# Okrio/CRUSE

Measured on AMD Instinct MI355X. Metric: spectrogram frames/sec training CRUSE 16kHz 20ms-hop at 1/2/4/8 MI355X, higher is better.
Workload: dtype bf16

## Files before the change

cruse_amd/_lib.py:

```python
from __future__ import annotations

import ctypes
import os

_HERE = os.path.dirname(os.path.abspath(__file__))
LIB_PATH = os.path.join(_HERE, "libcruse_hip.so")

ABI_VERSION = 14
PREC_F32, PREC_BF16X3, PREC_BF16, PREC_F16 = 0, 1, 2, 3
PREC_BY_NAME = {"f32": PREC_F32, "bf16x3": PREC_BF16X3, "bf16": PREC_BF16, "f16": PREC_F16}
DT_F32, DT_F16, DT_BF16 = 0, 1, 2

_T = {"p": ctypes.c_void_p, "i": ctypes.c_int, "f": ctypes.c_float, "q": ctypes.c_longlong, "d": ctypes.c_double, "c": ctypes.c_char_p,
      "z": ctypes.c_size_t, "Q": ctypes.c_ulonglong}

SIGNATURES = {
    "cruse_abi_version": ("", "i"),
    "cruse_last_error": ("", "s"),
    "cruse_set_option": ("cii", "i"),
    "cruse_get_option": ("cpp", "i"),
    "cruse_stft_fwd": ("piiiipppifp", "i"),
    "cruse_istft_fwd": ("ppiiiiipp", "i"),
    "cruse_istft_bwd": ("piiiiippp", "i"),
    "cruse_conv_gather": ("ppppiiiiiiiiiiiiiiip", "i"),
    "cruse_conv_scatter2": ("ppppiiiiiiiiiiiiip", "i"),
    "cruse_conv_gather_bnstats": ("ppppiiiiiiiiiipip", "i"),
    "cruse_conv_scatter2_bnstats": ("ppppiiiiiiiiipip", "i"),
    "cruse_conv_mfma_stamps": ("p", "i"),
    "cruse_conv_plan": ("i" * 17 + "p", "i"),
    "cruse_conv_gather_bnbwd": ("pppiiiiiiiiiiiipppppipiiip", "i"),
    "cruse_conv_scatter2_bnbwd": ("pppiiiiiiiiiipppppipiiip", "i"),
    "cruse_conv_wgrad_ws_bytes": ("iii", "z"),
    "cruse_conv_gather_bnbwd_in": ("pipppppp" + "iii" + "pppp" + "pp" + "iiiiiiiiiiii" + "pppppi" + "piip", "i"),
    "cruse_conv_scatter2_bnbwd_in": ("pipppppp" + "iii" + "pppp" + "pp" + "iiiiiiiiii" + "pppppi" + "piip", "i"),
    "cruse_conv_gather_bnin": ("ppiqffpppppppppppiiiiiiiiiipip", "i"),
    "cruse_conv_scatter2_bnin": ("ppiqffpppppppppppiiiiiiiiipip", "i"),
    "cruse_conv_wgrad": ("pppiiiiiiiiiiiipp", "i"),
    "cruse_channel_sum": ("pqiipp", "i"),
    "cruse_col_sum": ("pqiipp", "i"),
    "cruse_bn_stats": ("pqiipip", "i"),
    "cruse_bn_finalize_act_fwd": ("ppiqffpppppppppqiiip", "i"),
    "cruse_bn_finalize_act_fwd_c": ("ppiqffpppppippppqiiip", "i"),
    "cruse_bn_finalize": ("pqiffppppp", "i"),
    "cruse_bn_eval_stats": ("ppifppp", "i"),
    "cruse_bn_act_fwd": ("pppppppqiiip", "i"),
    "cruse_bn_act_bwd_reduce": ("ppppppqiiipip", "i"),
    "cruse_bn_act_bwd_apply": ("pppppppiqiiiiipipppp", "i"),
    "cruse_ln_fwd": ("ppppppppqiifiqqp", "i"),
    "cruse_ln_fwd_c": ("ppppppippqiifiqqp", "i"),
    "cruse_ln_bwd": ("pppppqiipppp", "i"),
    "cruse_gemm": ("iiiiipipipipiiiip", "i"),
    "cruse_gemm_bf16_nt": ("iiipqqpqqpqpiip", "i"),
    "cruse_gemm_bf16_slab_bytes": ("iii", "z"),
    "cruse_gemm_bf16_nt_slabs": ("iiipqqpqqpqipzp", "i"),
    "cruse_gemm_bf16_nt_slabs_cat": ("ipiippqqpqqpqipzp", "i"),
    "cruse_gemm_bf16_nt_groups": ("iiiippqqppqqqpqqpqip", "i"),
    "cruse_gemm_bf16_nt_seg": ("iiippqppqqpqpiiqqp", "i"),
    "cruse_cast_bf16": ("ppqp", "i"),
    "cruse_transpose_bf16": ("pqiqpqip", "i"),
    "cruse_ktile_bf16": ("piiqppp", "i"),
    "cruse_ktile_f16": ("piiqpp", "i"),
    "cruse_gemm_f16_nt": ("iiipqqpqqpqpp", "i"),
    "cruse_gemm_nt_out16": ("iiippqqppqqpqpiip", "i"),
    "cruse_gemm_bf16_nt_atr": ("iiipqipqqpqip", "i"),
    "cruse_gemm_f16x2_nt": ("iiipqqppqqpqpp", "i"),
    "cruse_ktile_f16_split": ("piiqppp", "i"),
    "cruse_cast_bf16_split": ("pppqp", "i"),
    "cruse_gemm_bf16x3_nt": ("iiippqqppqqpqpip", "i"),
    "cruse_gru_ws_bytes": ("iii", "z"),
    "cruse_gru_plan": ("iiiiip", "i"),
    "cruse_gru_seq_fwd": ("pppppppiiiiipp", "i"),
    "cruse_gru_seq_bwd": ("pppppiiiiipp", "i"),
    "cruse_gru_seq_fwd_on": ("pppppppiiiiippip", "i"),
    "cruse_gru_seq_bwd_on": ("pppppppiiiiippip", "i"),
    "cruse_gru_seq_fwd_ex": ("ppppppppqiiiiiiipipip", "i"),
    "cruse_gru_seq_fwd_gi16": ("pippppppiiiiiipipip", "i"),
    "cruse_gru_seq_bwd_ex": ("pppppppiiiiiiiiipipip", "i"),
    "cruse_gru_gate_grads": ("pppppqiiip", "i"),
    "cruse_gru_gate_grads_bf16": ("pppppqppqiip", "i"),
    "cruse_mask_loss_fwd": ("ppppqiiffpppppp", "i"),
    "cruse_mask_apply": ("pppqiippp", "i"),
    "cruse_mask_apply_bwd": ("pppppqiiipp", "i"),
    "cruse_mask_sdnr_fwd": ("pppppqiiiffpppp", "i"),
    "cruse_sisnr_fwd": ("ppiifpppp", "i"),
    "cruse_sisnr_bwd": ("pppiifpp", "i"),
    "cruse_wave_l1_mse": ("ppqifppp", "i"),
    "cruse_deepfilter_fwd": ("ppppiiiiippp", "i"),
    "cruse_deepfilter_bwd": ("ppppppiiiiippppp", "i"),
    "cruse_sigmoid_bwd": ("pppqp", "i"),
    "cruse_axpby": ("pppffqp", "i"),
    "cruse_adam_step": ("ppppqfffffifp", "i"),
    "cruse_adam_step_guarded": ("ppppqfffffiffppipppdpp", "i"),
    "cruse_step_health": ("ppppdp", "i"),
    "cruse_sumsq": ("pqpip", "i"),
    "cruse_conv2d_nchw": ("ppppiiiiiiiiiiiiiiiiiiipiip", "i"),
    "cruse_conv2d_nchw_wgrad": ("pppiiiiiiiiiiiiiiiiiip", "i"),
    "cruse_conv2d_nchw_wgrad_ex": ("ppppiiiiiiiiiiiiiiiiiip", "i"),
    "cruse_nchw_channel_sum": ("piiipip", "i"),
    "cruse_downsum_w": ("pqiipip", "i"),
    "cruse_upsample_w": ("pqiipip", "i"),
    "cruse_bn_nchw_stats": ("piiipip", "i"),
    "cruse_bn_nchw_fwd": ("ppppppiiiipip", "i"),
    "cruse_bn_nchw_bwd": ("pppppppiiiiipppppip", "i"),
    "cruse_bn_nchw_bwd_ex": ("pppppppiiiiipiipppppip", "i"),
    "cruse_conv2d_nchw_bnbwd": ("ppp" + "iiiiiii" + "iiiiiiii" + "ii" + "pppppp" + "i" + "pip" + "ip", "i"),
    "cruse_bn_nchw_stats_ex": ("piiipiip", "i"),
    "cruse_bn_nchw_fwd_train": ("ppiffpppiiiippppppip", "i"),
    "cruse_conv2d_nchw_ex": ("ppppp" + "iiiiiii" + "iiiiiiii" + "iiii" + "p" + "pi" + "ip", "i"),
    "cruse_add_nchw": ("pppqip", "i"),
    "cruse_cast_f16": ("ppqip", "i"),
    "cruse_stft_framed": ("ppiiiiiiiiifppp", "i"),
    "cruse_istft_framed": ("ppppiiiiiiiifipp", "i"),
    "cruse_mask_ops": ("ippppqfffppp", "i"),
    "cruse_polar": ("ippppqffppp", "i"),
    "cruse_rmse": ("ppqfppp", "i"),
    "cruse_c_rmse": ("ppiqffppp", "i"),
    "cruse_sisnr_plain_finalize": ("pifppp", "i"),
    "cruse_wo_male_spec": ("pppiqqqfffppp", "i"),
    "cruse_onepole_fir": ("piififpp", "i"),
    "cruse_snr_mix": ("pppiifppppp", "i"),
    "cruse_fir_causal": ("ppqiiipp", "i"),
    "cruse_stream_create_masked": ("ppi", "i"),
    "cruse_cu_census": ("piip", "i"),
    "cruse_cu_hog": ("iQp", "i"),
    "cruse_zero": ("pzp", "i"),
    "cruse_accum_f64": ("ppip", "i"),
    "cruse_counters_add": ("piqp", "i"),
    "cruse_stream_layout": ("iiiiip", "i"),
    "cruse_stream_tables": ("pp", "i"),
    "cruse_stream_encode": ("piiiiiipppppp", "i"),
    "cruse_stream_gru": ("piiiipiippfpiippiip", "i"),
    "cruse_stream_decode": ("piiiiiippfpppp", "i"),
    "cruse_stream_packet_layout": ("iiiiip", "i"),
    "cruse_stream_encode_n": ("piiiiiiiiipppppp", "i"),
    "cruse_stream_gru_proj_n": ("piiiiiipiippfppp", "i"),
    "cruse_stream_gru_rec_n": ("piiiiiippiippiip", "i"),
    "cruse_stream_decode_n": ("piiiiiiiiippfpppp", "i"),
    "cruse_stream_gru_f16": ("piiiipiippfpiipppiip", "i"),
    "cruse_stream_gru_proj_n_f16": ("piiiiiipiippfpppp", "i"),
    "cruse_stream_gru_rec_n_f16": ("piiiiiippiipppiip", "i"),
    "cruse_stream_encode_io": ("piiiiiipippppp", "i"),
    "cruse_stream_decode_io": ("piiiiiippfpppippp", "i"),
    "cruse_stream_encode_n_io": ("piiiiiiiiipippppp", "i"),
    "cruse_stream_decode_n_io": ("piiiiiiiiippfpppippp", "i"),
    "cruse_stream_resample_in": ("piipippipp", "i"),
    "cruse_stream_resample_out": ("piipppipipp", "i"),
    "cruse_stream_resample_in_n": ("piiiipippipp", "i"),
    "cruse_stream_resample_out_n": ("piiiipppipipp", "i"),
    "cruse_si_sdr": ("ppiipp", "i"),
    "cruse_stoi_layout": ("iip", "i"),
    "cruse_stoi_ws_bytes": ("ii", "z"),
    "cruse_stoi_tables": ("pp", "i"),
    "cruse_stoi": ("ppiippzpp", "i"),
    "cruse_biquad_ws_bytes": ("iii", "z"),
    "cruse_biquad_cascade": ("ppiiiiippp", "i"),
    "cruse_fftconv_spec_bytes": ("iii", "z"),
    "cruse_fftconv_ws_bytes": ("ii", "z"),
    "cruse_fftconv_prepare": ("piippzp", "i"),
    "cruse_fftconv_apply": ("piipziippzppp", "i"),
    "cruse_peak_scale": ("ppiifpp", "i"),
    "cruse_resample_poly": ("piiippppiiipiipp", "i"),
    "cruse_assemble_clips": ("pppiiipp", "i"),
}


def _load():
    if not os.path.exists(LIB_PATH):
        raise ImportError(
            f"{LIB_PATH} not found: the CRUSE HIP library must be built for gfx950 "
            "(run `python -c 'import __graft_entry__ as g; g.build()'`). There is no CPU fallback.")
    lib = ctypes.CDLL(LIB_PATH)
    for name, (args, res) in SIGNATURES.items():
        fn = getattr(lib, name)
        fn.argtypes = [_T[c] for c in args]
        fn.restype = ctypes.c_char_p if res == "s" else _T[res]
    if lib.cruse_abi_version() != ABI_VERSION:
        raise ImportError(f"libcruse_hip.so ABI version {lib.cruse_abi_version()} != {ABI_VERSION}")
    return lib


lib = _load()


def check(rc: int) -> None:
    if rc != 0:
        msg = lib.cruse_last_error()
        raise RuntimeError(f"cruse_hip error {rc}: {msg.decode() if msg else ''}")
```

cruse_amd/config.py:

```python
from __future__ import annotations

import contextlib
import os
from dataclasses import dataclass, field, fields, replace
from typing import Dict, Optional


@dataclass
class EngineConfig:
    overlap: bool = True
    defer_mask: int = 15
    inline_mask: int = 8
    fuse_bn_stats: bool = True
    fuse_bn_bwd_stats: bool = True
    gi_x3: Optional[int] = None
    gi_f16: int = 2
    fuse_bn_fwd: bool = True
    fuse_bn_bwd_apply: bool = True
    bf16_dy: bool = True
    bf16_de: bool = True
    gi_store_f16: bool = False
    dx_atr: bool = True
    pick_launch_stream: bool = True
    lib_options: Dict[str, int] = field(default_factory=dict)

    _ENV = {"overlap": ("CRUSE_OVERLAP", lambda v: v == "1"), "defer_mask": ("CRUSE_DEFER", int), "inline_mask": ("CRUSE_INLINE", int),
            "fuse_bn_stats": ("CRUSE_FUSE_BN_STATS", lambda v: v != "0"),
            
            "fuse_bn_bwd_stats": ("CRUSE_FUSE_BN_BWD", lambda v: v != "0"), 
            "gi_x3": ("CRUSE_GI_X3", int), "gi_f16": ("CRUSE_GI_F16", int), 
             
            "fuse_bn_fwd": ("CRUSE_FUSE_BN_FWD", lambda v: v != "0"), "fuse_bn_bwd_apply": ("CRUSE_FUSE_BN_BWD_APPLY", lambda v: v != "0"), "bf16_dy": ("CRUSE_BF16_DY", lambda v: v != "0"), "bf16_de": ("CRUSE_BF16_DE", lambda v: v != "0"),
            "pick_launch_stream": ("CRUSE_PICK_LAUNCH_STREAM", lambda v: v != "0"), "gi_store_f16": ("CRUSE_GI_STORE_F16", lambda v: v != "0"),
            "dx_atr": ("CRUSE_DX_ATR", lambda v: v != "0")}
    _LIB_ENV = {"CRUSE_GRU_BWD_RS": "gru_bwd_rs", "CRUSE_GRU_FWD_LEAN": "gru_fwd_lean", "CRUSE_GRU_WLO": "gru_wlo", "CRUSE_GRU_DBG": "gru_dbg",
                "CRUSE_GRU_TF": "gru_tf", "CRUSE_GRU_POLL_FWD": "gru_poll_fwd", "CRUSE_GRU_POLL_BWD": "gru_poll_bwd", "CRUSE_CM_KINT": "cm_kint",
                "CRUSE_CM_SWAP": "cm_swap", "CRUSE_CM_NW": "cm_nw", "CRUSE_PW_VALU": "pw_valu", "CRUSE_WG_DBG": "wg_dbg",
                "CRUSE_WG_RD": "wg_rd", "CRUSE_WG_GRID": "wg_grid"}

    @classmethod
    def from_env(cls, env=None) -> "EngineConfig":
        env = os.environ if env is None else env
        kw = {}
        for name, (var, conv) in cls._ENV.items():
            if var in env:
                kw[name] = conv(env[var])
        lib = {opt: int(env[var]) for var, opt in cls._LIB_ENV.items() if var in env}
        return cls(lib_options=lib, **kw)

    def non_default(self) -> dict:
        d = EngineConfig()
        return {f.name: getattr(self, f.name) for f in fields(self) if getattr(self, f.name) != getattr(d, f.name)}

    def copy(self, **kw) -> "EngineConfig":
        return replace(self, lib_options=dict(self.lib_options), **kw)


_ACTIVE = EngineConfig()


def get() -> EngineConfig:
    return _ACTIVE


@contextlib.contextmanager
def use(cfg: EngineConfig):
    global _ACTIVE
    from . import ops
    prev = _ACTIVE
    saved = {k: ops.get_option(k) for k in cfg.lib_options}
    _ACTIVE = cfg
    for k, v in cfg.lib_options.items():
        ops.set_option(k, v)
    try:
        yield cfg
    finally:
        _ACTIVE = prev
        for k, v in saved.items():
            ops.set_option(k, v)
```

cruse_amd/csrc/pointwise.hip:

```cpp
#include "common.h"
#include <stdlib.h>

namespace {

constexpr int RED_THREADS = 1024;
constexpr int CPR_MAXG = 3;

template <typename Fn>
__device__ __forceinline__ void channel_pair_reduce(long long rows, int C, int F, double* sums, Fn fn) {
    __shared__ double c1[64 * CPR_MAXG * 4], c2[64 * CPR_MAXG * 4];
    __shared__ double s1[256], s2[256];
    const int CF = C * F, ng = CF >> 2;
    const int tid = threadIdx.x, lane = tid & 63;
    for (int c = tid; c < C; c += blockDim.x) { s1[c] = 0.0; s2[c] = 0.0; }
    for (int i = tid; i < CF; i += blockDim.x) { c1[i] = 0.0; c2[i] = 0.0; }
    __syncthreads();
    float a[CPR_MAXG][4], b[CPR_MAXG][4];
#pragma unroll
    for (int g = 0; g < CPR_MAXG; ++g)
#pragma unroll
        for (int e = 0; e < 4; ++e) { a[g][e] = b[g][e] = 0.f; }
    auto flush = [&]() {
#pragma unroll
        for (int g = 0; g < CPR_MAXG; ++g) {
            const int q = lane + 64 * g;
            if (q < ng) {
#pragma unroll
                for (int e = 0; e < 4; ++e) {
                    atomicAdd(&c1[q * 4 + e], (double)a[g][e]);
                    atomicAdd(&c2[q * 4 + e], (double)b[g][e]);
                    a[g][e] = b[g][e] = 0.f;
                }
            }
        }
    };
    const int nw = blockDim.x >> 6;
    const long long wave = (long long)blockIdx.x * nw + (tid >> 6), nwave = (long long)gridDim.x * nw;
    int n = 0;
    for (long long r = wave; r < rows; r += 2 * nwave) {
        const bool two = r + nwave < rows;
#pragma unroll
        for (int g = 0; g < CPR_MAXG; ++g) {
            const int q = lane + 64 * g;
            if (q < ng) {
                float v[4], v2[4], w[4], w2[4];
                fn(r * CF + q * 4, g, v, v2);
                if (two) fn((r + nwave) * CF + q * 4, g, w, w2);
                else {
#pragma unroll
                    for (int e = 0; e < 4; ++e) { w[e] = 0.f; w2[e] = 0.f; }
                }
#pragma unroll
                for (int e = 0; e < 4; ++e) { a[g][e] += v[e] + w[e]; b[g][e] += v2[e] + w2[e]; }
            }
        }
        n += 2;
        if (n >= 32) { flush(); n = 0; }
    }
    flush();
    __syncthreads();
    for (int i = tid; i < CF; i += blockDim.x) {
        const int c = i / F;
        atomicAdd(&s1[c], c1[i]);
        atomicAdd(&s2[c], c2[i]);
    }
    __syncthreads();
    for (int c = tid; c < C; c += blockDim.x) {
        atomicAdd(&sums[c], s1[c]);
        atomicAdd(&sums[C + c], s2[c]);
    }
}

__global__ __launch_bounds__(RED_THREADS) void bn_stats_kernel(const float* y, long long rows, int C, int F, double* sums) {
    channel_pair_reduce(rows, C, F, sums, [&](long long i, int, float (&v)[4], float (&v2)[4]) {
        const float4 t = *reinterpret_cast<const float4*>(y + i);
        v[0] = t.x; v[1] = t.y; v[2] = t.z; v[3] = t.w;
#pragma unroll
        for (int e = 0; e < 4; ++e) v2[e] = v[e] * v[e];
    });
}

__global__ void bn_finalize_kernel(const double* sums, long long count, int C, float eps, float momentum,
                                   float* mean, float* rstd, float* rmean, float* rvar) {
    const int c = blockIdx.x * blockDim.x + threadIdx.x;
    if (c >= C) return;
    const double m = sums[c] / (double)count;
    double var = sums[C + c] / (double)count - m * m;
    if (var < 0.0) var = 0.0;
    mean[c] = (float)m;
    rstd[c] = (float)(1.0 / sqrt(var + (double)eps));
    if (rmean) {
        const double unb = count > 1 ? var * (double)count / (double)(count - 1) : var;
        rmean[c] = (float)((1.0 - momentum) * rmean[c] + momentum * m);
        rvar[c] = (float)((1.0 - momentum) * rvar[c] + momentum * unb);
    }
}

__global__ void bn_eval_stats_kernel(const float* rmean, const float* rvar, int C, float eps, float* mean, float* rstd) {
    const int c = blockIdx.x * blockDim.x + threadIdx.x;
    if (c >= C) return;
    mean[c] = rmean[c];
    rstd[c] = 1.0f / sqrtf(rvar[c] + eps);
}

__global__ __launch_bounds__(256) void bn_act_fwd_kernel(const float* y, const float* mean, const float* rstd,
                                                         const float* gamma, const float* beta, const float* skip,
                                                         float* out, long long rows, int C, int F, int relu) {
    extern __shared__ float tab[];
    for (int c = threadIdx.x; c < C; c += 256) {
        tab[c] = mean[c]; tab[C + c] = rstd[c]; tab[2 * C + c] = gamma[c]; tab[3 * C + c] = beta[c];
    }
    __syncthreads();
    const int CF = C * F;
    const long long n4 = rows * CF / 4;
    for (long long i = (long long)blockIdx.x * 256 + threadIdx.x; i < n4; i += (long long)gridDim.x * 256) {
        const float4 v = reinterpret_cast<const float4*>(y)[i];
        float4 s = make_float4(0.f, 0.f, 0.f, 0.f);
        if (skip) s = reinterpret_cast<const float4*>(skip)[i];
        const int j = (int)((i * 4) % CF);
        float in[4] = {v.x, v.y, v.z, v.w};
        float sk[4] = {s.x, s.y, s.z, s.w};
        float o[4];
#pragma unroll
        for (int e = 0; e < 4; ++e) {
            const int c = (j + e) / F;
            float t = (in[e] - tab[c]) * tab[C + c] * tab[2 * C + c] + tab[3 * C + c];
            if (relu) t = fmaxf(t, 0.f);
            o[e] = t + sk[e];
        }
        reinterpret_cast<float4*>(out)[i] = make_float4(o[0], o[1], o[2], o[3]);
    }
}

__device__ __forceinline__ void store_copy4(void* base, long long elem, const float o0, const float o1, const float o2, const float o3,
                                            const int copy_f16) {
    if (copy_f16) {
        typedef __attribute__((ext_vector_type(4))) _Float16 f16x4_;
        const f16x4_ b = {(_Float16)o0, (_Float16)o1, (_Float16)o2, (_Float16)o3};
        *reinterpret_cast<f16x4_*>(reinterpret_cast<_Float16*>(base) + elem) = b;
    } else {
        typedef __attribute__((ext_vector_type(4))) __bf16 bf16x4_;
        const bf16x4_ b = {(__bf16)o0, (__bf16)o1, (__bf16)o2, (__bf16)o3};
        *reinterpret_cast<bf16x4_*>(reinterpret_cast<__bf16*>(base) + elem) = b;
    }
}

__global__ __launch_bounds__(256) void bn_fin_act_fwd_kernel(const float* y, const double* sums, int nrep, double inv_count, double unb,
                                                             float eps, float momentum, const float* gamma,
                                                             const float* beta, const float* skip, float* out, __bf16* out_bf,
                                                             float* mean_o, float* rstd_o, float* rmean, float* rvar,
                                                             long long rows, int C, int F, int relu, int copy_f16) {
    extern __shared__ float tab[];
    for (int c = threadIdx.x; c < C; c += 256) {
        double t1 = 0.0, t2 = 0.0;
        for (int r = 0; r < nrep; ++r) { t1 += sums[(long long)r * 2 * C + c]; t2 += sums[(long long)r * 2 * C + C + c]; }
        const double m = t1 * inv_count;
        double var = t2 * inv_count - m * m;
        if (var < 0.0) var = 0.0;
        const float mf = (float)m, rs = (float)(1.0 / sqrt(var + (double)eps));
        tab[c] = mf; tab[C + c] = rs; tab[2 * C + c] = gamma[c]; tab[3 * C + c] = beta[c];
        if (blockIdx.x == 0) {
            mean_o[c] = mf; rstd_o[c] = rs;
            if (rmean) {
                rmean[c] = (float)((1.0 - momentum) * rmean[c] + momentum * m);
                rvar[c] = (float)((1.0 - momentum) * rvar[c] + momentum * var * unb);
            }
        }
    }
    __syncthreads();
    const int CF = C * F;
    if (CF <= 64 * CPR_MAXG * 4) {
        const int lane = threadIdx.x & 63, ng = CF >> 2;
        float pm[CPR_MAXG][4], pr[CPR_MAXG][4], pg[CPR_MAXG][4], pb[CPR_MAXG][4];
#pragma unroll
        for (int g = 0; g < CPR_MAXG; ++g)
#pragma unroll
            for (int e = 0; e < 4; ++e) {
                const int col = (lane + 64 * g) * 4 + e;
                const int c = col < CF ? col / F : 0;
                pm[g][e] = tab[c]; pr[g][e] = tab[C + c]; pg[g][e] = tab[2 * C + c]; pb[g][e] = tab[3 * C + c];
            }
        const long long wave = (long long)blockIdx.x * 4 + (threadIdx.x >> 6), nwave = (long long)gridDim.x * 4;
        for (long long r = wave; r < rows; r += nwave) {
            float4 vv[CPR_MAXG], ss[CPR_MAXG];
            if (skip) {
#pragma unroll
                for (int g = 0; g < CPR_MAXG; ++g) {
                    const int q = lane + 64 * g;
                    if (q < ng) { vv[g] = *reinterpret_cast<const float4*>(y + r * CF + q * 4); ss[g] = *reinterpret_cast<const float4*>(skip + r * CF + q * 4); }
                }
            } else {
#pragma unroll
                for (int g = 0; g < CPR_MAXG; ++g) {
                    const int q = lane + 64 * g;
                    if (q < ng) { vv[g] = *reinterpret_cast<const float4*>(y + r * CF + q * 4); ss[g] = make_float4(0.f, 0.f, 0.f, 0.f); }
                }
            }
#pragma unroll
            for (int g = 0; g < CPR_MAXG; ++g) {
                const int q = lane + 64 * g;
                if (q < ng) {
                    const long long i = r * CF + q * 4;
                    const float in[4] = {vv[g].x, vv[g].y, vv[g].z, vv[g].w}, sk[4] = {ss[g].x, ss[g].y, ss[g].z, ss[g].w};
                    float o[4];
#pragma unroll
                    for (int e = 0; e < 4; ++e) {
                        float t = (in[e] - pm[g][e]) * pr[g][e] * pg[g][e] + pb[g][e];
                        if (relu) t = fmaxf(t, 0.f);
                        o[e] = t + sk[e];
                    }
                    *reinterpret_cast<float4*>(out + i) = make_float4(o[0], o[1], o[2], o[3]);
                    if (out_bf) store_copy4(out_bf, i, o[0], o[1], o[2], o[3], copy_f16);
                }
            }
        }
        return;
    }
    const long long n4 = rows * CF / 4;
    for (long long i = (long long)blockIdx.x * 256 + threadIdx.x; i < n4; i += (long long)gridDim.x * 256) {
        const float4 v = reinterpret_cast<const float4*>(y)[i];
        float4 s = make_float4(0.f, 0.f, 0.f, 0.f);
        if (skip) s = reinterpret_cast<const float4*>(skip)[i];
        const int j = (int)((i * 4) % CF);
        const float in[4] = {v.x, v.y, v.z, v.w};
        const float sk[4] = {s.x, s.y, s.z, s.w};
        float o[4];
#pragma unroll
        for (int e = 0; e < 4; ++e) {
            const int c = (j + e) / F;
            float t = (in[e] - tab[c]) * tab[C + c] * tab[2 * C + c] + tab[3 * C + c];
            if (relu) t = fmaxf(t, 0.f);
            o[e] = t + sk[e];
        }
        reinterpret_cast<float4*>(out)[i] = make_float4(o[0], o[1], o[2], o[3]);
        if (out_bf) store_copy4(out_bf, i * 4, o[0], o[1], o[2], o[3], copy_f16);
    }
}

__global__ __launch_bounds__(RED_THREADS) void bn_act_bwd_reduce_kernel(const float* dout, const float* y, const float* mean,
                                                                const float* rstd, const float* gamma,
                                                                const float* beta, long long rows, int C, int F,
                                                                int relu, double* sums) {
    __shared__ float tab[4][256];
    float pm[CPR_MAXG][4], pr[CPR_MAXG][4], pg[CPR_MAXG][4], pb[CPR_MAXG][4];
    const int lane = threadIdx.x & 63;
    for (int c = threadIdx.x; c < C; c += blockDim.x) {
        tab[0][c] = mean[c]; tab[1][c] = rstd[c]; tab[2][c] = gamma[c]; tab[3][c] = beta[c];
    }
    __syncthreads();
#pragma unroll
    for (int g = 0; g < CPR_MAXG; ++g)
#pragma unroll
        for (int e = 0; e < 4; ++e) {
            const int col = (lane + 64 * g) * 4 + e;
            const int c = col < C * F ? col / F : 0;
            pm[g][e] = tab[0][c]; pr[g][e] = tab[1][c]; pg[g][e] = tab[2][c]; pb[g][e] = tab[3][c];
        }
    channel_pair_reduce(rows, C, F, sums, [&](long long i, int g, float (&v)[4], float (&v2)[4]) {
        const float4 yy = *reinterpret_cast<const float4*>(y + i);
        const float4 dd = *reinterpret_cast<const float4*>(dout + i);
        const float yv[4] = {yy.x, yy.y, yy.z, yy.w}, dv[4] = {dd.x, dd.y, dd.z, dd.w};
#pragma unroll
        for (int e = 0; e < 4; ++e) {
            const float xh = (yv[e] - pm[g][e]) * pr[g][e];
            float gr = dv[e];
            if (relu && !(xh * pg[g][e] + pb[g][e] > 0.f)) gr = 0.f;
            v[e] = gr; v2[e] = gr * xh;
        }
    });
}

__global__ __launch_bounds__(256) void bn_act_bwd_apply_kernel(const float* dout, const float* y, const float* mean,
                                                               const float* rstd, const float* gamma,
                                                               const float* beta, const double* sums, int nrep, long long rows,
                                                               int C, int F, int relu, int training, float* dy, int dy_bf16,
                                                               int dout_bf16, float* dgamma, float* dbeta, float* dbias) {
    __shared__ float tab[6][256];
    const double cnt = (double)rows * F;
    const int tid = threadIdx.x, lane = tid & 63;
    const int CF = C * F, ng = CF >> 2;
    for (int c = tid; c < C; c += 256) {
        double sg = 0.0, sgx = 0.0;
        for (int r = 0; r < nrep; ++r) { sg += sums[(size_t)r * 2 * C + c]; sgx += sums[(size_t)r * 2 * C + C + c]; }
        tab[0][c] = mean[c]; tab[1][c] = rstd[c]; tab[2][c] = gamma[c]; tab[3][c] = beta[c];
        tab[4][c] = training ? (float)(sg / cnt) : 0.f;
        tab[5][c] = training ? (float)(sgx / cnt) : 0.f;
        if (blockIdx.x == 0) {
            if (dgamma) dgamma[c] += (float)sgx;
            if (dbeta) dbeta[c] += (float)sg;
            if (dbias && !training) dbias[c] += gamma[c] * rstd[c] * (float)sg;
        }
    }
    __syncthreads();
    float pm[CPR_MAXG][4], pr[CPR_MAXG][4], pg[CPR_MAXG][4], pb[CPR_MAXG][4], p1[CPR_MAXG][4], p2[CPR_MAXG][4];
#pragma unroll
    for (int g = 0; g < CPR_MAXG; ++g)
#pragma unroll
        for (int e = 0; e < 4; ++e) {
            const int col = (lane + 64 * g) * 4 + e;
            const int c = col < CF ? col / F : 0;
            pm[g][e] = tab[0][c]; pr[g][e] = tab[1][c]; pg[g][e] = tab[2][c]; pb[g][e] = tab[3][c];
            p1[g][e] = tab[4][c]; p2[g][e] = tab[5][c];
        }
    const long long wave = (long long)blockIdx.x * 4 + (tid >> 6), nwave = (long long)gridDim.x * 4;
    for (long long r = wave; r < rows; r += nwave) {
        float4 vv[CPR_MAXG], dv[CPR_MAXG];
        if (dout_bf16) {
#pragma unroll
            for (int g = 0; g < CPR_MAXG; ++g) {
                const int q = lane + 64 * g;
                if (q < ng) {
                    const long long i = r * CF + q * 4;
                    vv[g] = *reinterpret_cast<const float4*>(y + i);
                    const float2 w2 = *reinterpret_cast<const float2*>(reinterpret_cast<const __bf16*>(dout) + i);
                    const unsigned w0 = __float_as_uint(w2.x), w1 = __float_as_uint(w2.y);
                    dv[g] = make_float4(__uint_as_float(w0 << 16), __uint_as_float(w0 & 0xffff0000u), __uint_as_float(w1 << 16),
                                        __uint_as_float(w1 & 0xffff0000u));
                }
            }
        } else {
#pragma unroll
            for (int g = 0; g < CPR_MAXG; ++g) {
                const int q = lane + 64 * g;
                if (q < ng) {
                    const long long i = r * CF + q * 4;
                    vv[g] = *reinterpret_cast<const float4*>(y + i);
                    dv[g] = *reinterpret_cast<const float4*>(dout + i);
                }
            }
        }
#pragma unroll
        for (int g = 0; g < CPR_MAXG; ++g) {
            const int q = lane + 64 * g;
            if (q < ng) {
                const long long i = r * CF + q * 4;
                const float in[4] = {vv[g].x, vv[g].y, vv[g].z, vv[g].w}, dd[4] = {dv[g].x, dv[g].y, dv[g].z, dv[g].w};
                float o[4];
#pragma unroll
                for (int e = 0; e < 4; ++e) {
                    const float xh = (in[e] - pm[g][e]) * pr[g][e];
                    float gr = dd[e];
                    if (relu && !(xh * pg[g][e] + pb[g][e] > 0.f)) gr = 0.f;
                    o[e] = pg[g][e] * pr[g][e] * (gr - p1[g][e] - xh * p2[g][e]);
                }
                if (dy_bf16) {
                    typedef __attribute__((ext_vector_type(4))) __bf16 bf16x4_;
                    bf16x4_ h;
                    h[0] = (__bf16)o[0]; h[1] = (__bf16)o[1]; h[2] = (__bf16)o[2]; h[3] = (__bf16)o[3];
                    *reinterpret_cast<bf16x4_*>(reinterpret_cast<__bf16*>(dy) + i) = h;
                } else {
                    *reinterpret_cast<float4*>(dy + i) = make_float4(o[0], o[1], o[2], o[3]);
                }
            }
        }
    }
}

constexpr int LN_MAXE = 16;

__device__ __forceinline__ int ln_perm(int c, int H, int g) {
    if (g <= 1) return c;
    const int Hg = H / g;
    return (c % Hg) * g + c / Hg;
}

__global__ __launch_bounds__(256) void ln_fwd_kernel(const float* x, const float* gamma, const float* beta,
                                                     const float* res, float* y, float* mean, float* rstd,
                                                     long long rows, int H, int g, float eps) {
    const int lane = threadIdx.x & 63;
    const long long wave = (long long)blockIdx.x * 4 + (threadIdx.x >> 6);
    const long long nwave = (long long)gridDim.x * 4;
    for (long long r = wave; r < rows; r += nwave) {
        float v[LN_MAXE];
        float s = 0.f;
#pragma unroll
        for (int e = 0; e < LN_MAXE; ++e) {
            const int c = lane + 64 * e;
            v[e] = c < H ? x[r * H + c] : 0.f;
            s += v[e];
        }
        const float m = wave_sum(s) / (float)H;
        float q = 0.f;
#pragma unroll
        for (int e = 0; e < LN_MAXE; ++e) {
            const int c = lane + 64 * e;
            const float d = c < H ? v[e] - m : 0.f;
            q += d * d;
        }
        const float rs = 1.0f / sqrtf(wave_sum(q) / (float)H + eps);
        if (lane == 0) { if (mean) mean[r] = m; if (rstd) rstd[r] = rs; }
#pragma unroll
        for (int e = 0; e < LN_MAXE; ++e) {
            const int c = lane + 64 * e;
            if (c < H) {
                const int p = ln_perm(c, H, g);
                float o = (v[e] - m) * rs * gamma[p] + beta[p];
                if (res) o += res[r * H + p];
                y[r * H + p] = o;
            }
        }
    }
}

__global__ __launch_bounds__(256) void ln_bwd_kernel(const float* dy, const float* x, const float* mean,
                                                     const float* rstd, const float* gamma, long long rows, int H,
                                                     int g, float* dx, float* dgamma, float* dbeta) {
    __shared__ float sdg[1024], sdb[1024];
    const int lane = threadIdx.x & 63;
    for (int c = threadIdx.x; c < H; c += 256) { sdg[c] = 0.f; sdb[c] = 0.f; }
    __syncthreads();
    const long long wave = (long long)blockIdx.x * 4 + (threadIdx.x >> 6);
    const long long nwave = (long long)gridDim.x * 4;
    float adg[LN_MAXE], adb[LN_MAXE];
    int perm[LN_MAXE];
    float gm[LN_MAXE];
#pragma unroll
    for (int e = 0; e < LN_MAXE; ++e) {
        adg[e] = 0.f; adb[e] = 0.f;
        const int c = lane + 64 * e;
        perm[e] = c < H ? ln_perm(c, H, g) : 0;
        gm[e] = c < H ? gamma[perm[e]] : 0.f;
    }
    for (long long r = wave; r < rows; r += nwave) {
        const float m = mean[r], rs = rstd[r];
        float xh[LN_MAXE], gd[LN_MAXE];
        float s1 = 0.f, s2 = 0.f;
#pragma unroll
        for (int e = 0; e < LN_MAXE; ++e) {
            const int c = lane + 64 * e;
            if (c < H) {
                const float d = dy[r * H + perm[e]];
                xh[e] = (x[r * H + c] - m) * rs;
                gd[e] = d * gm[e];
                adg[e] += d * xh[e];
                adb[e] += d;
                s1 += gd[e];
                s2 += gd[e] * xh[e];
            } else { xh[e] = 0.f; gd[e] = 0.f; }
        }
        const float m1 = wave_sum(s1) / (float)H, m2 = wave_sum(s2) / (float)H;
#pragma unroll
        for (int e = 0; e < LN_MAXE; ++e) {
            const int c = lane + 64 * e;
            if (c < H) dx[r * H + c] = rs * (gd[e] - m1 - xh[e] * m2);
        }
    }
#pragma unroll
    for (int e = 0; e < LN_MAXE; ++e) {
        const int c = lane + 64 * e;
        if (c < H) { atomicAdd(&sdg[perm[e]], adg[e]); atomicAdd(&sdb[perm[e]], adb[e]); }
    }
    __syncthreads();
    for (int c = threadIdx.x; c < H; c += 256) {
        if (dgamma) atomicAdd(&dgamma[c], sdg[c]);
        if (dbeta) atomicAdd(&dbeta[c], sdb[c]);
    }
}

constexpr int LNV_MAXQ = 4;
constexpr int LNV_NR = 2;

struct RowSeg { int len; long long stride, off; };
__device__ __forceinline__ long long seg_row(const RowSeg& sg, long long r) {
    if (sg.len == 0) return r;
    const long long q = r / sg.len;
    return q * sg.stride + sg.off + (r - q * sg.len);
}

__global__ __launch_bounds__(256) void ln_fwd_vec_kernel(const float* x, const float* gamma, const float* beta,
                                                         const float* res, float* y, __bf16* y_bf, float* mean, float* rstd,
                                                         long long rows, int H, float eps, RowSeg sg, int copy_f16) {
    const int lane = threadIdx.x & 63, nq = H >> 2;
    const long long wave = (long long)blockIdx.x * 4 + (threadIdx.x >> 6);
    const long long nwave = (long long)gridDim.x * 4;
    float4 gm[LNV_MAXQ], bt[LNV_MAXQ];
#pragma unroll
    for (int e = 0; e < LNV_MAXQ; ++e) {
        const int q = lane + 64 * e;
        gm[e] = q < nq ? reinterpret_cast<const float4*>(gamma)[q] : make_float4(0.f, 0.f, 0.f, 0.f);
        bt[e] = q < nq ? reinterpret_cast<const float4*>(beta)[q] : make_float4(0.f, 0.f, 0.f, 0.f);
    }
    for (long long r0 = wave * LNV_NR; r0 < rows; r0 += nwave * LNV_NR) {
        float4 v[LNV_NR][LNV_MAXQ], rv[LNV_NR][LNV_MAXQ];
        float s[LNV_NR], m[LNV_NR], qq[LNV_NR];
#pragma unroll
        for (int k = 0; k < LNV_NR; ++k) {
            const long long rl = r0 + k, r = seg_row(sg, rl < rows ? rl : rows - 1);
            s[k] = 0.f;
#pragma unroll
            for (int e = 0; e < LNV_MAXQ; ++e) {
                const int q = lane + 64 * e;
                const bool ok = q < nq && rl < rows;
                v[k][e] = ok ? reinterpret_cast<const float4*>(x + r * H)[q] : make_float4(0.f, 0.f, 0.f, 0.f);
                rv[k][e] = (ok && res) ? reinterpret_cast<const float4*>(res + r * H)[q] : make_float4(0.f, 0.f, 0.f, 0.f);
                s[k] += (v[k][e].x + v[k][e].y) + (v[k][e].z + v[k][e].w);
            }
// ... 161 lines not shown

__global__ void sigmoid_bwd_kernel(const float* dmask, const float* mask, float* dlogit, long long n) {
    for (long long i = (long long)blockIdx.x * blockDim.x + threadIdx.x; i < n; i += (long long)gridDim.x * blockDim.x) {
        const float m = mask[i];
        dlogit[i] = dmask[i] * m * (1.f - m);
    }
}

__global__ void axpby_kernel(float* out, const float* x, const float* y, float a, float b, long long n) {
    for (long long i = (long long)blockIdx.x * blockDim.x + threadIdx.x; i < n; i += (long long)gridDim.x * blockDim.x)
        out[i] = a * x[i] + (y ? b * y[i] : 0.f);
}

__global__ void accum_f64_kernel(double* acc, const double* x, int n) {
    const int i = blockIdx.x * blockDim.x + threadIdx.x;
    if (i < n) acc[i] += x[i];
}
__global__ void step_health_kernel(unsigned* gru_status, const double* loss_sum, unsigned* health, double* loss_acc,
                                   double loss_scale) {
    if (threadIdx.x != 0 || blockIdx.x != 0) return;
    unsigned to = 0u;
    if (gru_status) {
        to = __hip_atomic_load(gru_status, __ATOMIC_RELAXED, __HIP_MEMORY_SCOPE_AGENT) != 0u ? 1u : 0u;
        if (to) __hip_atomic_store(gru_status, 0u, __ATOMIC_RELAXED, __HIP_MEMORY_SCOPE_AGENT);
    }
    const double l = loss_sum ? *loss_sum : 0.0;
    health[0] = to;
    health[1] = isfinite(l) ? 0u : 1u;
    if (loss_acc && isfinite(l)) *loss_acc += l * loss_scale;
}
struct CounterPtrs { long long* p[32]; };
__global__ void counters_add_kernel(CounterPtrs c, int n, long long v) {
    const int i = threadIdx.x;
    if (i < n) *c.p[i] += v;
}

__global__ void adam_kernel(float* p, const float* g, float* m, float* v, long long n, float lr, float b1, float b2,
                            float eps, float wd, int step, float gscale, float max_norm,
                            const double* gsumsq, const unsigned* skip_flag, int n_skip_words, const double* loss_check,
                            unsigned* skipped, const double* loss_sum, double loss_scale, double* loss_acc) {
    const int step_eff = max(1, step - (skipped ? (int)*skipped : 0));
    const float bc1 = (float)(1.0 - pow((double)b1, (double)step_eff));
    const float bc2_sqrt = (float)sqrt(1.0 - pow((double)b2, (double)step_eff));
    bool skip = false;
    for (int i = 0; i < n_skip_words; ++i)
        if (skip_flag[i] != 0u) skip = true;
    if (loss_check && !isfinite(*loss_check)) skip = true;
    if (gsumsq) {
        const double norm = sqrt(*gsumsq) * (double)gscale;
        if (!isfinite(norm)) skip = true;
        else if (max_norm > 0.f) {
            const double coef = (double)max_norm / (norm + 1e-6);
            if (coef < 1.0) gscale = (float)((double)gscale * coef);
        }
    }
    if (skip) {
        if (skipped && blockIdx.x == 0 && threadIdx.x == 0) {
            atomicAdd(skipped, 1u);
            for (int i = 0; i < n_skip_words && n_skip_words > 1; ++i)
                if (skip_flag[i] != 0u) atomicAdd(skipped + 1 + i, 1u);
        }
        return;
    }
    if (loss_acc && loss_sum && blockIdx.x == 0 && threadIdx.x == 0) { loss_acc[0] += *loss_sum * loss_scale; loss_acc[1] += 1.0; }
    for (long long i = (long long)blockIdx.x * blockDim.x + threadIdx.x; i < n; i += (long long)gridDim.x * blockDim.x) {
        float gi = g[i] * gscale;
        const float pi = p[i];
        if (wd != 0.f) gi += wd * pi;
        const float mi = b1 * m[i] + (1.f - b1) * gi;
        const float vi = b2 * v[i] + (1.f - b2) * gi * gi;
        m[i] = mi; v[i] = vi;
        const float denom = sqrtf(vi) / bc2_sqrt + eps;
        p[i] = pi - (lr / bc1) * (mi / denom);
    }
}

__global__ __launch_bounds__(1024) void sumsq_kernel(const float* x, long long n, double* out) {
    __shared__ double part[16];
    double acc = 0.0;
    const long long n4 = n >> 2;
    const float4* x4 = reinterpret_cast<const float4*>(x);
    for (long long i = (long long)blockIdx.x * blockDim.x + threadIdx.x; i < n4; i += (long long)gridDim.x * blockDim.x) {
        const float4 a = x4[i];
        acc += (double)(a.x * a.x + a.y * a.y) + (double)(a.z * a.z + a.w * a.w);
    }
    if (blockIdx.x == 0 && threadIdx.x < (n & 3)) { const float a = x[(n4 << 2) + threadIdx.x]; acc += (double)a * a; }
    acc = wave_sum_d(acc);
    if ((threadIdx.x & 63) == 0) part[threadIdx.x >> 6] = acc;
    __syncthreads();
    if (threadIdx.x < 64) {
        double t = threadIdx.x < (blockDim.x >> 6) ? part[threadIdx.x] : 0.0;
        t = wave_sum_d(t);
        if (threadIdx.x == 0) atomicAdd(out, t);
    }
}

inline int grid_for(long long n, int per_block, int cap = 4096) {
    long long g = (n + per_block - 1) / per_block;
    if (g < 1) g = 1;
    if (g > cap) g = cap;
    return (int)g;
}

}

extern "C" int cruse_cast_bf16_split(const float* x, void* y, void* y_lo, long long n, void* stream);

#define ST(s) ((hipStream_t)(s))

extern "C" int cruse_bn_stats(const float* y, long long rows, int C, int F, double* sums, int zeroed, void* stream) {
    CRUSE_REQUIRE(rows > 0 && C > 0 && C <= 256 && F > 0, CRUSE_E_SHAPE, "bn_stats: bad shape rows=%lld C=%d F=%d", rows, C, F);
    CRUSE_REQUIRE((C * F) % 4 == 0 && C * F <= 768, CRUSE_E_SHAPE, "bn_stats: C*F=%d must be a multiple of 4 and <= 768", C * F);
    if (!zeroed) { int zrc = cruse_zero_async(sums, 2 * C * sizeof(double), ST(stream), "bn_stats memset"); if (zrc) return zrc; }
    hipLaunchKernelGGL(bn_stats_kernel, dim3(grid_for(rows, 64, 256)), dim3(RED_THREADS), 0, ST(stream), y, rows, C, F, sums);
    CRUSE_LAUNCH_CHECK("bn_stats");
    return CRUSE_OK;
}

extern "C" int cruse_bn_finalize(const double* sums, long long count, int C, float eps, float momentum,
                                 float* mean, float* rstd, float* running_mean, float* running_var, void* stream) {
    CRUSE_REQUIRE(count > 0 && C > 0, CRUSE_E_SHAPE, "bn_finalize: bad shape");
    CRUSE_REQUIRE((running_mean == nullptr) == (running_var == nullptr), CRUSE_E_SHAPE, "bn_finalize: running stats");
    hipLaunchKernelGGL(bn_finalize_kernel, dim3(cdiv(C, 64)), dim3(64), 0, ST(stream), sums, count, C, eps, momentum,
                       mean, rstd, running_mean, running_var);
    CRUSE_LAUNCH_CHECK("bn_finalize");
    return CRUSE_OK;
}

extern "C" int cruse_bn_eval_stats(const float* running_mean, const float* running_var, int C, float eps,
                                   float* mean, float* rstd, void* stream) {
    CRUSE_REQUIRE(C > 0, CRUSE_E_SHAPE, "bn_eval_stats: bad shape");
    hipLaunchKernelGGL(bn_eval_stats_kernel, dim3(cdiv(C, 64)), dim3(64), 0, ST(stream), running_mean, running_var, C,
                       eps, mean, rstd);
    CRUSE_LAUNCH_CHECK("bn_eval_stats");
    return CRUSE_OK;
}

extern "C" int cruse_bn_act_fwd(const float* y, const float* mean, const float* rstd, const float* gamma,
                                const float* beta, const float* skip, float* out,
                                long long rows, int C, int F, int relu, void* stream) {
    CRUSE_REQUIRE(rows > 0 && C > 0 && F > 0, CRUSE_E_SHAPE, "bn_act_fwd: bad shape");
    CRUSE_REQUIRE((C * F) % 4 == 0, CRUSE_E_ALIGN, "bn_act_fwd: C*F=%d must be a multiple of 4", C * F);
    hipLaunchKernelGGL(bn_act_fwd_kernel, dim3(grid_for(rows * C * F / 4, 1024)), dim3(256), 4 * C * sizeof(float),
                       ST(stream), y, mean, rstd, gamma, beta, skip, out, rows, C, F, relu);
    CRUSE_LAUNCH_CHECK("bn_act_fwd");
    return CRUSE_OK;
}

extern "C" int cruse_bn_finalize_act_fwd_c(const float* y, const double* sums, int sum_replicas, long long count, float eps, float momentum,
                                           const float* gamma, const float* beta, const float* skip, float* out, void* out_copy, int copy_dtype,
                                           float* mean, float* rstd, float* running_mean, float* running_var,
                                           long long rows, int C, int F, int relu, void* stream);

extern "C" int cruse_bn_finalize_act_fwd(const float* y, const double* sums, int sum_replicas, long long count, float eps, float momentum,
                                         const float* gamma, const float* beta, const float* skip, float* out, void* out_bf16,
                                         float* mean, float* rstd, float* running_mean, float* running_var,
                                         long long rows, int C, int F, int relu, void* stream) {
    return cruse_bn_finalize_act_fwd_c(y, sums, sum_replicas, count, eps, momentum, gamma, beta, skip, out, out_bf16, CRUSE_DT_BF16, mean, rstd,
                                       running_mean, running_var, rows, C, F, relu, stream);
}

extern "C" int cruse_bn_finalize_act_fwd_c(const float* y, const double* sums, int sum_replicas, long long count, float eps, float momentum,
                                           const float* gamma, const float* beta, const float* skip, float* out, void* out_bf16, int copy_dtype,
                                           float* mean, float* rstd, float* running_mean, float* running_var,
                                           long long rows, int C, int F, int relu, void* stream) {
    CRUSE_REQUIRE(copy_dtype == CRUSE_DT_BF16 || copy_dtype == CRUSE_DT_F16, CRUSE_E_DTYPE, "bn_finalize_act_fwd: copy_dtype %d (bf16 or f16)", copy_dtype);
    CRUSE_REQUIRE(rows > 0 && C > 0 && C <= 256 && F > 0 && count > 0 && sum_replicas >= 1, CRUSE_E_SHAPE, "bn_finalize_act_fwd: bad shape");
    CRUSE_REQUIRE((C * F) % 4 == 0, CRUSE_E_ALIGN, "bn_finalize_act_fwd: C*F=%d must be a multiple of 4", C * F);
    CRUSE_REQUIRE((running_mean == nullptr) == (running_var == nullptr) && mean && rstd, CRUSE_E_SHAPE, "bn_finalize_act_fwd: statistics");
    const double unb = count > 1 ? (double)count / (double)(count - 1) : 1.0;
    const bool rowwise = C * F <= 64 * CPR_MAXG * 4 && (C * F) % 4 == 0;
    hipLaunchKernelGGL(bn_fin_act_fwd_kernel, dim3(rowwise ? grid_for(rows, 8, 2048) : grid_for(rows * C * F / 4, 1024)), dim3(256), 4 * C * sizeof(float), ST(stream),
                       y, sums, sum_replicas, 1.0 / (double)count, unb, eps, momentum, gamma, beta, skip, out, (__bf16*)out_bf16, mean, rstd, running_mean,
                       running_var, rows, C, F, relu, copy_dtype == CRUSE_DT_F16 ? 1 : 0);
    CRUSE_LAUNCH_CHECK("bn_finalize_act_fwd");
    return CRUSE_OK;
}

extern "C" int cruse_bn_act_bwd_reduce(const float* dout, const float* y, const float* mean, const float* rstd,
                                       const float* gamma, const float* beta, long long rows, int C, int F,
                                       int relu, double* sums, int zeroed, void* stream) {
    CRUSE_REQUIRE(rows > 0 && C > 0 && C <= 256 && F > 0, CRUSE_E_SHAPE, "bn_act_bwd_reduce: bad shape");
    CRUSE_REQUIRE((C * F) % 4 == 0 && C * F <= 768, CRUSE_E_SHAPE, "bn_act_bwd_reduce: C*F=%d must be a multiple of 4 and <= 768", C * F);
    if (!zeroed) { int zrc = cruse_zero_async(sums, 2 * C * sizeof(double), ST(stream), "bn_act_bwd_reduce memset"); if (zrc) return zrc; }
    hipLaunchKernelGGL(bn_act_bwd_reduce_kernel, dim3(grid_for(rows, 64, 256)), dim3(RED_THREADS), 0, ST(stream), dout, y, mean,
                       rstd, gamma, beta, rows, C, F, relu, sums);
    CRUSE_LAUNCH_CHECK("bn_act_bwd_reduce");
    return CRUSE_OK;
}

extern "C" int cruse_bn_act_bwd_apply(const float* dout, const float* y, const float* mean, const float* rstd,
                                      const float* gamma, const float* beta, const double* sums, int sum_replicas,
                                      long long rows, int C, int F, int relu, int training, int dout_dtype,
                                      void* dy, int dy_dtype, float* dgamma, float* dbeta, float* dbias, void* stream) {
    CRUSE_REQUIRE((dy_dtype == CRUSE_DT_F32 || dy_dtype == CRUSE_DT_BF16) && (dout_dtype == CRUSE_DT_F32 || dout_dtype == CRUSE_DT_BF16),
                  CRUSE_E_DTYPE, "bn_act_bwd_apply: dout_dtype %d / dy_dtype %d (f32 or bf16)", dout_dtype, dy_dtype);
    CRUSE_REQUIRE(rows > 0 && C > 0 && C <= 256 && F > 0 && sum_replicas >= 1, CRUSE_E_SHAPE, "bn_act_bwd_apply: bad shape");
    CRUSE_REQUIRE((C * F) % 4 == 0 && C * F <= 768, CRUSE_E_SHAPE,
                  "bn_act_bwd_apply: C*F=%d must be a multiple of 4 and <= 768", C * F);
    hipLaunchKernelGGL(bn_act_bwd_apply_kernel, dim3(grid_for(rows, 8, 2048)), dim3(256), 0, ST(stream), dout, y,
                       mean, rstd, gamma, beta, sums, sum_replicas, rows, C, F, relu, training, (float*)dy,
                       dy_dtype == CRUSE_DT_BF16 ? 1 : 0, dout_dtype == CRUSE_DT_BF16 ? 1 : 0, dgamma, dbeta, dbias);
    CRUSE_LAUNCH_CHECK("bn_act_bwd_apply");
    return CRUSE_OK;
}

extern "C" int cruse_ln_fwd_c(const float* x, const float* gamma, const float* beta, const float* res,
                              float* y, void* y_copy, int copy_dtype, float* mean, float* rstd, long long rows, int H, int interleave_g,
                              float eps, int seg_len, long long seg_stride, long long seg_off, void* stream);

extern "C" int cruse_ln_fwd(const float* x, const float* gamma, const float* beta, const float* res,
                            float* y, void* y_bf16, float* mean, float* rstd, long long rows, int H, int interleave_g,
                            float eps, int seg_len, long long seg_stride, long long seg_off, void* stream) {
    return cruse_ln_fwd_c(x, gamma, beta, res, y, y_bf16, CRUSE_DT_BF16, mean, rstd, rows, H, interleave_g, eps, seg_len, seg_stride, seg_off,
                          stream);
}

extern "C" int cruse_ln_fwd_c(const float* x, const float* gamma, const float* beta, const float* res,
                              float* y, void* y_bf16, int copy_dtype, float* mean, float* rstd, long long rows, int H, int interleave_g,
                              float eps, int seg_len, long long seg_stride, long long seg_off, void* stream) {
    CRUSE_REQUIRE(copy_dtype == CRUSE_DT_BF16 || copy_dtype == CRUSE_DT_F16, CRUSE_E_DTYPE, "ln_fwd: copy_dtype %d (bf16 or f16)", copy_dtype);
    CRUSE_REQUIRE(seg_len >= 0 && (seg_len == 0 || (seg_stride >= seg_len && seg_off >= 0 && rows % seg_len == 0)), CRUSE_E_SHAPE,
                  "ln_fwd: bad row segments (len %d stride %lld off %lld, rows %lld)", seg_len, seg_stride, seg_off, rows);
    const RowSeg sg = {seg_len, seg_stride, seg_off};
    CRUSE_REQUIRE(rows > 0 && H > 0 && H <= 64 * LN_MAXE, CRUSE_E_SHAPE, "ln_fwd: H=%d must be in 1..%d", H, 64 * LN_MAXE);
    CRUSE_REQUIRE(interleave_g >= 1 && H % interleave_g == 0, CRUSE_E_SHAPE, "ln_fwd: groups=%d must divide H=%d", interleave_g, H);
    const bool vec = interleave_g == 1 && H % 4 == 0 && H <= 256 * LNV_MAXQ &&
                     ((((uintptr_t)x | (uintptr_t)y | (uintptr_t)gamma | (uintptr_t)beta | (uintptr_t)res) & 15) == 0);
    const bool bf_inline = vec && y_bf16 && (((uintptr_t)y_bf16 & 7) == 0);
    if (vec)
        hipLaunchKernelGGL(ln_fwd_vec_kernel, dim3(grid_for(rows, 16, 2048)), dim3(256), 0, ST(stream), x, gamma, beta,
                           res, y, bf_inline ? (__bf16*)y_bf16 : nullptr, mean, rstd, rows, H, eps, sg, copy_dtype == CRUSE_DT_F16 ? 1 : 0);
    else {
        CRUSE_REQUIRE(seg_len == 0, CRUSE_E_SHAPE, "ln_fwd: row segments need the vector form (one group, H %% 4 == 0, aligned)");
        hipLaunchKernelGGL(ln_fwd_kernel, dim3(grid_for(rows, 4, 2048)), dim3(256), 0, ST(stream), x, gamma, beta, res, y,
                           mean, rstd, rows, H, interleave_g, eps);
    }
    CRUSE_LAUNCH_CHECK("ln_fwd");
    CRUSE_REQUIRE(seg_len == 0 || !y_bf16 || bf_inline, CRUSE_E_ALIGN, "ln_fwd: row segments need an 8-byte aligned bf16 copy");
    CRUSE_REQUIRE(copy_dtype == CRUSE_DT_BF16 || !y_bf16 || bf_inline, CRUSE_E_DTYPE, "ln_fwd: the f16 copy needs the vector form (one group)");
    if (y_bf16 && !bf_inline) return cruse_cast_bf16_split(y, y_bf16, nullptr, rows * H, stream);
    return CRUSE_OK;
}

static int lnb_grid() { return cruse_opt("lnb_grid", 512); }

static int ln_bwd_impl(const float* dy, const float* x, const float* mean, const float* rstd,
                       const float* gamma, long long rows, int H, int interleave_g,
                       float* dx, float* dgamma, float* dbeta, int seg_len, long long seg_stride, long long seg_off, void* stream) {
    CRUSE_REQUIRE(rows > 0 && H > 0 && H <= 64 * LN_MAXE, CRUSE_E_SHAPE, "ln_bwd: H=%d must be in 1..%d", H, 64 * LN_MAXE);
    CRUSE_REQUIRE(interleave_g >= 1 && H % interleave_g == 0, CRUSE_E_SHAPE, "ln_bwd: groups=%d must divide H=%d", interleave_g, H);
    CRUSE_REQUIRE(seg_len >= 0 && (seg_len == 0 || (seg_stride >= seg_len && seg_off >= 0 && rows % seg_len == 0)), CRUSE_E_SHAPE,
                  "ln_bwd: bad row segments (len %d stride %lld off %lld, rows %lld)", seg_len, seg_stride, seg_off, rows);
    const RowSeg sg = {seg_len, seg_stride, seg_off};
    const bool vec = interleave_g == 1 && H % 4 == 0 && H <= 256 * LNV_MAXQ &&
                     ((((uintptr_t)dy | (uintptr_t)x | (uintptr_t)dx | (uintptr_t)gamma) & 15) == 0);
    if (vec && H <= 768)
        hipLaunchKernelGGL((ln_bwd_vec_kernel<3, 2>), dim3(grid_for(rows, 16, lnb_grid())), dim3(256), 0, ST(stream), dy, x, mean,
                           rstd, gamma, rows, H, dx, dgamma, dbeta, sg);
    else if (vec)
        hipLaunchKernelGGL((ln_bwd_vec_kernel<4, 1>), dim3(grid_for(rows, 16, lnb_grid())), dim3(256), 0, ST(stream), dy, x, mean,
                           rstd, gamma, rows, H, dx, dgamma, dbeta, sg);
    else {
        CRUSE_REQUIRE(seg_len == 0, CRUSE_E_SHAPE, "ln_bwd: row segments need the vector form (one group, H %% 4 == 0, aligned)");
        hipLaunchKernelGGL(ln_bwd_kernel, dim3(grid_for(rows, 32, 1024)), dim3(256), 0, ST(stream), dy, x, mean, rstd,
                           gamma, rows, H, interleave_g, dx, dgamma, dbeta);
    }
    CRUSE_LAUNCH_CHECK("ln_bwd");
    return CRUSE_OK;
}

extern "C" int cruse_ln_bwd(const float* dy, const float* x, const float* mean, const float* rstd,
                            const float* gamma, long long rows, int H, int interleave_g,
                            float* dx, float* dgamma, float* dbeta, void* stream) {
    return ln_bwd_impl(dy, x, mean, rstd, gamma, rows, H, interleave_g, dx, dgamma, dbeta, 0, 0, 0, stream);
}

extern "C" int cruse_mask_loss_fwd(const float* mask, const float* nre, const float* nim, const float* cmag,
                                   long long rows, int Fn, int Fs, float alpha, float beta,
                                   double* loss_sum, float* dmask, float* dlogit, float* est_re, float* est_im,
                                   void* stream) {
    CRUSE_REQUIRE(rows > 0 && Fn > 0 && Fs >= Fn, CRUSE_E_SHAPE, "mask_loss: bad shape rows=%lld Fn=%d Fs=%d", rows, Fn, Fs);
    { int zrc = cruse_zero_async(loss_sum, sizeof(double), ST(stream), "mask_loss memset"); if (zrc) return zrc; }
    hipLaunchKernelGGL(mask_loss_kernel, dim3(grid_for(rows * Fs, 2048, 2048)), dim3(256), 0, ST(stream), mask, nre, nim,
                       cmag, rows, Fn, Fs, alpha, beta, loss_sum, dmask, dlogit, est_re, est_im);
    CRUSE_LAUNCH_CHECK("mask_loss");
    return CRUSE_OK;
}

extern "C" int cruse_sigmoid_bwd(const float* dmask, const float* mask, float* dlogit, long long n, void* stream) {
    CRUSE_REQUIRE(n > 0, CRUSE_E_SHAPE, "sigmoid_bwd: n=%lld", n);
    hipLaunchKernelGGL(sigmoid_bwd_kernel, dim3(grid_for(n, 1024)), dim3(256), 0, ST(stream), dmask, mask, dlogit, n);
    CRUSE_LAUNCH_CHECK("sigmoid_bwd");
    return CRUSE_OK;
}

extern "C" int cruse_axpby(float* out, const float* x, const float* y, float a, float b, long long n, void* stream) {
    CRUSE_REQUIRE(n > 0, CRUSE_E_SHAPE, "axpby: n=%lld", n);
    hipLaunchKernelGGL(axpby_kernel, dim3(grid_for(n, 1024)), dim3(256), 0, ST(stream), out, x, y, a, b, n);
    CRUSE_LAUNCH_CHECK("axpby");
    return CRUSE_OK;
}

extern "C" int cruse_accum_f64(double* acc, const double* x, int n, void* stream) {
    CRUSE_REQUIRE(n > 0, CRUSE_E_SHAPE, "accum_f64: n=%d", n);
    hipLaunchKernelGGL(accum_f64_kernel, dim3(cdiv(n, 64)), dim3(64), 0, ST(stream), acc, x, n);
    CRUSE_LAUNCH_CHECK("accum_f64");
    return CRUSE_OK;
}

extern "C" int cruse_step_health(unsigned* gru_status, const double* loss_sum, unsigned* health, double* loss_acc,
                                 double loss_scale, void* stream) {
    CRUSE_REQUIRE(health != nullptr, CRUSE_E_SHAPE, "step_health: health is required");
    hipLaunchKernelGGL(step_health_kernel, dim3(1), dim3(64), 0, ST(stream), gru_status, loss_sum, health, loss_acc, loss_scale);
    CRUSE_LAUNCH_CHECK("step_health");
    return CRUSE_OK;
}

extern "C" int cruse_counters_add(long long* const* counters, int n, long long v, void* stream) {
    CRUSE_REQUIRE(n > 0 && n <= 32, CRUSE_E_SHAPE, "counters_add: n=%d (1..32)", n);
    CounterPtrs c = {};
    for (int i = 0; i < n; ++i) c.p[i] = counters[i];
    hipLaunchKernelGGL(counters_add_kernel, dim3(1), dim3(64), 0, ST(stream), c, n, v);
    CRUSE_LAUNCH_CHECK("counters_add");
    return CRUSE_OK;
}

extern "C" int cruse_zero(void* p, size_t bytes, void* stream) {
    CRUSE_REQUIRE(bytes % 4 == 0, CRUSE_E_SHAPE, "zero: %zu bytes is not a multiple of 4", bytes);
    return cruse_zero_async(p, bytes, ST(stream), "zero");
}

extern "C" int cruse_adam_step_guarded(float* p, const float* g, float* m, float* v, long long n,
                                       float lr, float beta1, float beta2, float eps, float weight_decay,
                                       int step, float grad_scale, float max_norm, const double* gsumsq,
                                       const unsigned* skip_flag, int n_skip_words, const double* loss_check,
                                       unsigned* skipped, const double* loss_sum, double loss_scale, double* loss_acc,
                                       void* stream) {
    CRUSE_REQUIRE(n > 0 && step >= 1, CRUSE_E_SHAPE, "adam_step: n=%lld step=%d", n, step);
    CRUSE_REQUIRE(n_skip_words >= 0 && n_skip_words <= 8 && (n_skip_words == 0 || skip_flag != nullptr), CRUSE_E_SHAPE,
                  "adam_step: n_skip_words=%d (0..8, with skip_flag)", n_skip_words);
    CRUSE_REQUIRE(max_norm <= 0.f || gsumsq != nullptr, CRUSE_E_SHAPE, "adam_step: max_norm needs the gradient sum of squares");
    hipLaunchKernelGGL(adam_kernel, dim3(grid_for(n, 1024)), dim3(256), 0, ST(stream), p, g, m, v, n, lr, beta1, beta2,
                       eps, weight_decay, step, grad_scale, max_norm, gsumsq, skip_flag,
                       skip_flag ? n_skip_words : 0, loss_check, skipped, loss_sum, loss_scale, loss_acc);
    CRUSE_LAUNCH_CHECK("adam_step");
    return CRUSE_OK;
}

extern "C" int cruse_adam_step(float* p, const float* g, float* m, float* v, long long n,
                               float lr, float beta1, float beta2, float eps, float weight_decay,
                               int step, float grad_scale, void* stream) {
    return cruse_adam_step_guarded(p, g, m, v, n, lr, beta1, beta2, eps, weight_decay, step, grad_scale, 0.f, nullptr,
                                   nullptr, 0, nullptr, nullptr, nullptr, 1.0, nullptr, stream);
}

// ... 9 lines not shown
```

cruse_amd/model/cruse_net.py:

```python
from __future__ import annotations

from typing import Dict, List, Optional, Tuple

import contextlib
import torch
import torch.nn as nn

from .. import config, ops, streams

DEFAULT_PREC = "f32"


_KEEP_EVENTS: list = []


def record_event(stream) -> "torch.cuda.Event":
    e = torch.cuda.Event()
    e.record(stream)
    if torch.cuda.is_current_stream_capturing():
        if len(_KEEP_EVENTS) > 200000:
            del _KEEP_EVENTS[:100000]
        _KEEP_EVENTS.append(e)
    return e

# ... 340 lines not shown
    Hg = H // g
    rows = B * T
    hooks = [pre_done] if pre_done is not None else []

    def run_bwd(dout_h, w_hh, coef, z, an=None, dg_slabs=3):
        if hooks:
            hooks.pop()()
        slot_, zeroed = STEP_SCRATCH.take(B, g, Hg, slot)
        return SIDE.release_around(lambda: ops.gru_seq_bwd(dout_h, w_hh, coef, z, B, T, g, Hg, prec, slot=slot_,
                                                           xcd_rot=xcd_rot, an=an, want_dgi=an is not None, dg_slabs=dg_slabs,
                                                           zeroed=zeroed))

    def dinp_buffer(dout_h, need_dinp, last):
        if not need_dinp:
            return None, False
        if last:
            if dx_accum and dx_ready is not None:
                dx_ready()
            return dx, dx_accum
        return torch.empty(B, T, H, device=dout_h.device, dtype=torch.float32), False

    def layer_bwd_bf16(dout_h, lname, inp, h, coef, an, z, need_dinp, last):
        names = [f"{prefix}{lname}.{i}." for i in range(g)]
        w_hh = [P[nm + "weight_hh_l0"] for nm in names]
        bias_ih = [G[nm + "bias_ih_l0"] for nm in names]
        bias_hh = [G[nm + "bias_hh_l0"] for nm in names]
        ldT = (rows + 63) // 64 * 64
        dh = run_bwd(dout_h, w_hh, coef, z)
        dx_atr = bool(config.get().dx_atr) and Hg % 64 == 0 and need_dinp and g == 1
        dgi, dgT, ldT = ops.gru_gate_grads_bf16(dh, coef, an, rows, g, Hg, bias_ih, bias_hh, want_dgi=not dx_atr)
        early = early_T.pop(lname, None)
        if early is not None:
            inpT, hpT = early
        else:
            inpT = torch.empty(ldT // 64, H, 64, device=dh.device, dtype=torch.bfloat16)
            hpT = torch.empty(ldT // 64, H, 64, device=dh.device, dtype=torch.bfloat16)

        def weight_grads():
            if early is None:
                ops.transpose_bf16(inp, rows, H, out=inpT)
                ops.transpose_bf16(h, rows, H, shift_T=T, out=hpT)
            ka, kb = 4 * H * 64, H * 64
            for i, nm in enumerate(names):
                a0, b0 = 4 * i * Hg * 64, i * Hg * 64
                g_ih, g_hh = G[nm + "weight_ih_l0"], G[nm + "weight_hh_l0"]
                sk = _splitk_bf16(6 * Hg, Hg, ldT)
                if (abs(sk) > 1
                        and g_hh.data_ptr() == g_ih.data_ptr() + 4 * 3 * Hg * Hg):
                    ops.gemm_bf16_nt_cat([3 * Hg, 2 * Hg, Hg], Hg, ldT, dgT, [4 * i * Hg, 4 * i * Hg, 4 * i * Hg + 3 * Hg], 64,
                                         [inpT, hpT, hpT], b0, 64, g_ih, 0, Hg, sk, a_kstride=ka, b_kstride=kb)
                    continue
                ops.gemm_bf16_nt(3 * Hg, Hg, ldT, dgT, a0, 64, inpT, b0, 64, G[nm + "weight_ih_l0"], 0, Hg,
                                 accumulate=True, splitk=_splitk_bf16(3 * Hg, Hg, ldT), slabs=True, a_kstride=ka, b_kstride=kb)
                ops.gemm_bf16_nt(2 * Hg, Hg, ldT, dgT, a0, 64, hpT, b0, 64, G[nm + "weight_hh_l0"], 0, Hg,
                                 accumulate=True, splitk=_splitk_bf16(2 * Hg, Hg, ldT), slabs=True, a_kstride=ka, b_kstride=kb)
                ops.gemm_bf16_nt(Hg, Hg, ldT, dgT, a0 + 3 * Hg * 64, 64, hpT, b0, 64, G[nm + "weight_hh_l0"],
                                 2 * Hg * Hg, Hg, accumulate=True, splitk=_splitk_bf16(Hg, Hg, ldT), slabs=True, a_kstride=ka,
                                 b_kstride=kb)

        early_leaf = last and not defer_last
        if early_leaf:
            SIDE.run(weight_grads, dgT, h, inp, inpT, hpT, dh, lane=2)
        dinp, acc_dx = dinp_buffer(dout_h, need_dinp, last)
        stack = ctx.get("w_ts", {}).get((lname, "stack"))
        if need_dinp and g > 1 and stack is not None:
            ops.gemm_bf16_nt_groups(rows, Hg, stack.shape[1] * 64, g, dgi, None, 3 * H, 3 * Hg, stack, None, 64, stack[0].numel(), dinp, H, Hg,
                                    accumulate=acc_dx, b_kstride=Hg * 64)
        elif need_dinp:
            for i, nm in enumerate(names):
                w_t = ctx.get("w_ts", {}).get((lname, i))
                if w_t is None:
                    w_t = ops.transpose_bf16(P[nm + "weight_ih_l0"], 3 * Hg, Hg)
                if dgi is None:
                    ops.gemm_bf16_nt_atr(rows, Hg, 3 * Hg, dgT, 4 * i * Hg * 64, g * 4 * Hg * 64, ldT // 64, w_t, 0, 64, dinp, i * Hg, H,
                                         accumulate=acc_dx, b_kstride=Hg * 64)
                    continue
                ops.gemm_bf16_nt(rows, Hg, w_t.shape[0] * 64, dgi, i * 3 * Hg, 3 * H, w_t, 0, 64, dinp, i * Hg, H,
                                 accumulate=acc_dx, b_kstride=Hg * 64)
        if early_leaf:
            pass
        elif last and defer_last:
            SIDE.defer(weight_grads, dgT, h, inp, inpT, hpT, dh, kind=0xffff, lane=2)
        elif last:
            SIDE.run(weight_grads, dgT, h, inp, inpT, hpT, dh, lane=2)
        else:
            SIDE.defer(weight_grads, dgT, h, inp, inpT, hpT, dh, kind=4, lane=2)
        return dinp

    def layer_bwd(dout_h, lname, inp, h, coef, an, z, need_dinp, last):
        if _bf16_gemm_path(prec, Hg):
            return layer_bwd_bf16(dout_h, lname, inp, h, coef, an, z, need_dinp, last)
        w_hh = [P[f"{prefix}{lname}.{i}.weight_hh_l0"] for i in range(g)]
        dh = run_bwd(dout_h, w_hh, coef, z)
        dgi, dgh = ops.gru_gate_grads(dh, coef, an, rows, g, Hg, prec)
        sk = _splitk(3 * Hg, Hg, rows)

        def weight_grads():
            for i in range(g):
                nm = f"{prefix}{lname}.{i}."
                ops.gemm(True, False, 3 * Hg, Hg, rows, dgh, i * 3 * Hg, 3 * H, h, i * Hg, H, G[nm + "weight_hh_l0"], 0,
                         Hg, accumulate=True, splitk=sk, b_shift_T=T, prec=prec)
                ops.col_sum(dgh, i * 3 * Hg, rows, 3 * Hg, 3 * H, G[nm + "bias_hh_l0"])
                ops.gemm(True, False, 3 * Hg, Hg, rows, dgi, i * 3 * Hg, 3 * H, inp, i * Hg, H, G[nm + "weight_ih_l0"], 0,
                         Hg, accumulate=True, splitk=sk, prec=prec)
                ops.col_sum(dgi, i * 3 * Hg, rows, 3 * Hg, 3 * H, G[nm + "bias_ih_l0"])

        dinp, acc_dx = dinp_buffer(dout_h, need_dinp, last)
        if need_dinp:
            for i in range(g):
                ops.gemm(False, False, rows, Hg, 3 * Hg, dgi, i * 3 * Hg, 3 * H,
                         P[f"{prefix}{lname}.{i}.weight_ih_l0"], 0, Hg, dinp, i * Hg, H, accumulate=acc_dx, prec=prec)
        if last and defer_last:
            SIDE.defer(weight_grads, dgi, dgh, h, inp, kind=0xffff, lane=2)
        elif last:
            SIDE.run(weight_grads, dgi, dgh, h, inp, lane=2)
        else:
            SIDE.defer(weight_grads, dgi, dgh, h, inp, kind=4, lane=2)
        return dinp

    early_T = {}
    if "T1" in ctx:
        early_T["gru_list1"], early_T["gru_list2"] = ctx["T1"], ctx["T2"]
    elif _bf16_gemm_path(prec, Hg) and SIDE.enabled:
        ldT1 = (rows + 63) // 64 * 64
        x1T = torch.empty(ldT1 // 64, H, 64, device=dout.device, dtype=torch.bfloat16)
        h1T = torch.empty(ldT1 // 64, H, 64, device=dout.device, dtype=torch.bfloat16)
        early_T["gru_list1"] = (x1T, h1T)

        def early_transposes(x1=ctx["x"], h1=ctx["h1"]):
            ops.transpose_bf16(x1, rows, H, out=x1T)
            ops.transpose_bf16(h1, rows, H, shift_T=T, out=h1T)
        SIDE.defer(early_transposes, x1T, h1T, kind=4, lane=2)
    dh2 = ops.ln_bwd(dout, ctx["h2"], ctx["m2"], ctx["s2"], P[prefix + "ln2.weight"], rows, H, 1,
                     G[prefix + "ln2.weight"], G[prefix + "ln2.bias"])
    dl1 = layer_bwd(dh2, "gru_list2", ctx["l1"], ctx["h2"], ctx["c2"], ctx["a2"], ctx["z2"], True, False)
    dh1 = ops.ln_bwd(dl1, ctx["h1"], ctx["m1"], ctx["s1"], P[prefix + "ln1.weight"], rows, H, g,
                     G[prefix + "ln1.weight"], G[prefix + "ln1.bias"])
    layer_bwd(dh1, "gru_list1", ctx["x"], ctx["h1"], ctx["c1"], ctx["a1"], ctx["z1"], need_dx, True)


BN_EPS = 1e-5
BN_MOMENTUM = 0.1


_PENDING_COUNTERS = []


def _flush_counters():
    if _PENDING_COUNTERS:
        ops.counters_add(list(_PENDING_COUNTERS), 1)
        _PENDING_COUNTERS.clear()


def _bn_act(y, rows, C, F, P, Bf, name, training, update_running, skip=None, sums=None, out_bf16=None):
    gamma, beta = P[name + ".weight"], P[name + ".bias"]
    if training:
        if sums is None:
            sums = ops.bn_stats(y, rows, C, F)
        rm = Bf[name + ".running_mean"] if update_running else None
        rv = Bf[name + ".running_var"] if update_running else None
        if update_running:
            _PENDING_COUNTERS.append(Bf[name + ".num_batches_tracked"])
        return ops.bn_finalize_act_fwd(y, sums, rows * F, BN_EPS, BN_MOMENTUM, gamma, beta, skip, rows, C, F, relu=True,
                                       running_mean=rm, running_var=rv, out_bf16=out_bf16)
    mean, rstd = ops.bn_eval_stats(Bf[name + ".running_mean"], Bf[name + ".running_var"], BN_EPS)
    return ops.bn_act_fwd(y, mean, rstd, gamma, beta, skip, rows, C, F, relu=True), mean, rstd


def unet2_forward(x: torch.Tensor, P: Dict[str, torch.Tensor], Bf: Dict[str, torch.Tensor], ch, groups: int,
                  prec, training: bool, save: bool = True, update_running: bool = True, dec_mode: str = "transposed"):
    if dec_mode not in ("transposed", "upsample"):
        raise RuntimeError(f"unet2_forward: unknown dec_mode {dec_mode!r}")
    ups = dec_mode == "upsample"
    if x.dim() != 4 or x.shape[1] != ch[0]:
        raise RuntimeError(f"unet_2 expects [B,{ch[0]},T,F], got {tuple(x.shape)}")
    if ch[0] != 1:
        raise RuntimeError("cruse_amd unet_2 supports ch[0] == 1 (magnitude input) only")
    B, _, T, F0 = x.shape
    L = len(ch) - 1
    if F0 % (1 << L) != 0:
        raise RuntimeError(f"unet_2: {F0} input bins are not divisible by 2**{L} (the network runs on in_feat//2*2 bins)")
    rows = B * T
    Fk = [F0 >> k for k in range(L + 1)]
    ctx = dict(B=B, T=T, F=Fk, ch=tuple(ch), L=L, prec=prec, training=training, x=x)
    cur = x
    _PENDING_COUNTERS.clear()
    ys, es, ss, stats = [None], [x], [None], [None]
    fz = (training and save and config.get().fuse_bn_fwd and config.get().fuse_bn_stats
          and all(ch[k] * Fk[k] <= 640 for k in range(1, L + 1)))
    dev = x.device

    def virtual(y_, sums_, C, F, name, add=None):
        mean_ = torch.empty(C, device=dev, dtype=torch.float32); rstd_ = torch.empty(C, device=dev, dtype=torch.float32)
        rm = Bf[name + ".running_mean"] if update_running else None
        rv = Bf[name + ".running_var"] if update_running else None
        if update_running:
            _PENDING_COUNTERS.append(Bf[name + ".num_batches_tracked"])
        return ops.BnIn(y_, sums_, ops.BN_STAT_REPLICAS, rows * F, BN_EPS, BN_MOMENTUM, P[name + ".weight"], P[name + ".bias"], mean_, rstd_,
                        rm, rv, add=add)
    pend = None
    e_bf = None
    for k in range(1, L + 1):
        if pend is not None:
            y, sums = ops.conv_gather_bnin(pend, P[f"conv{k}.weight"], P[f"conv{k}.bias"], B, T, ch[k - 1], Fk[k - 1], ch[k], Fk[k], KT=2, S=2,
                                           pad=1, prec=prec, publish=True, copy_bf16=es[k - 1], want_sums=True)
        elif training and config.get().fuse_bn_stats:
            y, sums = ops.conv_gather_bnstats(cur, P[f"conv{k}.weight"], P[f"conv{k}.bias"], B, T, ch[k - 1], Fk[k - 1], ch[k],
                                              Fk[k], KT=2, S=2, pad=1, prec=prec)
        else:
            y, sums = ops.conv_gather(cur, P[f"conv{k}.weight"], P[f"conv{k}.bias"], B, T, ch[k - 1], Fk[k - 1], ch[k], Fk[k],
                                      KT=2, S=2, pad=1, prec=prec), None
        s = torch.empty(B, T, ch[k], Fk[k], device=x.device, dtype=torch.float32)
        if fz and k < L and ops.bnin_eligible(prec, ch[k], ch[k + 1]) and ops.bnin_eligible(prec, ch[k], ch[k]):
            pend = virtual(y, sums, ch[k], Fk[k], f"bn{k}")
            e = torch.empty(B, T, ch[k], Fk[k], device=dev, dtype=torch.bfloat16)
            mean, rstd = pend.mean, pend.rstd

            def skip_conv(bn=pend, s=s, k=k):
                ops.conv_gather_bnin(bn, P[f"skip_connect_{k}.weight"], None, B, T, ch[k], Fk[k], ch[k], Fk[k], KT=1, S=1, pad=1,
                                     prec=prec, out=s)
            SIDE.defer(skip_conv, y, s, kind=1, lane=1)
        else:
            pend = None
            e_bf = None
            if k == L and training and _gi_takes_bf16_copy(prec, ch[L] * Fk[L] // groups):
                e_bf = torch.empty(rows * ch[L] * Fk[L], device=x.device,
                                   dtype=torch.float16 if _gi_f16(prec, ch[L] * Fk[L] // groups, 0) else torch.bfloat16)
            e, mean, rstd = _bn_act(y, rows, ch[k], Fk[k], P, Bf, f"bn{k}", training, update_running, sums=sums, out_bf16=e_bf)

            def skip_conv(e=e, s=s, k=k):
                ops.conv_gather(e, P[f"skip_connect_{k}.weight"], None, B, T, ch[k], Fk[k], ch[k], Fk[k], KT=1, S=1, pad=1,
                                out=s, prec=prec)
            SIDE.defer(skip_conv, e, s, kind=1, lane=1)
        ys.append(y); es.append(e); ss.append(s); stats.append((mean, rstd))
        cur = e
    H = ch[L] * Fk[L]
    late = []
    u, gctx = ggru_forward(cur.view(B, T, H), P, "gru.", groups, prec, residual=ss[L].view(B, T, H), save=save,
                           residual_ready=SIDE.join, late_leaves=late, x_bf16=e_bf)
    u = u.view(B, T, ch[L], Fk[L])
    SIDE.join()
    for fn, keep in late:
        SIDE.run(fn, *keep, lane=2)
    us, vs, dstats, uus = {L: u}, {}, {}, {}
    pend = None
    for k in range(L, 1, -1):
        if ups:
            uus[k] = ops.upsample_w(u, rows * ch[k], Fk[k], 2).view(B, T, ch[k], Fk[k - 1])
            if training and config.get().fuse_bn_stats:
                v, sums = ops.conv_gather_bnstats(uus[k], P[f"conv{k}_t.weight"], P.get(f"conv{k}_t.bias"), B, T, ch[k], Fk[k - 1], ch[k - 1],
                                                  Fk[k - 1], KT=1, S=1, pad=1, prec=prec)
            else:
                v, sums = ops.conv_gather(uus[k], P[f"conv{k}_t.weight"], P.get(f"conv{k}_t.bias"), B, T, ch[k], Fk[k - 1], ch[k - 1],
                                          Fk[k - 1], KT=1, S=1, pad=1, prec=prec), None
        elif pend is not None:
            v, sums = ops.conv_scatter2_bnin(pend, P[f"conv{k}_t.weight"], P[f"conv{k}_t.bias"], B, T, ch[k], Fk[k], ch[k - 1], KT=1, pad=0,
                                             prec=prec, publish=True, copy_bf16=us[k], want_sums=True)
        elif training and config.get().fuse_bn_stats:
            v, sums = ops.conv_scatter2_bnstats(u, P[f"conv{k}_t.weight"], P[f"conv{k}_t.bias"], B, T, ch[k], Fk[k], ch[k - 1],
                                                KT=1, pad=0, prec=prec)
        else:
            v, sums = ops.conv_scatter2(u, P[f"conv{k}_t.weight"], P[f"conv{k}_t.bias"], B, T, ch[k], Fk[k], ch[k - 1], KT=1,
                                        pad=0, prec=prec), None
        if fz and not ups and k - 1 >= 2 and ops.bnin_eligible(prec, ch[k - 1], ch[k - 2]):
            pend = virtual(v, sums, ch[k - 1], Fk[k - 1], f"bn{k}_t", add=ss[k - 1])
            u = torch.empty(B, T, ch[k - 1], Fk[k - 1], device=dev, dtype=torch.bfloat16)
            mean, rstd = pend.mean, pend.rstd
        else:
            pend = None
            u, mean, rstd = _bn_act(v, rows, ch[k - 1], Fk[k - 1], P, Bf, f"bn{k}_t", training, update_running, skip=ss[k - 1],
                                    sums=sums)
        vs[k] = v; dstats[k] = (mean, rstd); us[k - 1] = u
    if ups:
        uus[1] = ops.upsample_w(u, rows * ch[1], Fk[1], 2).view(B, T, ch[1], Fk[0])
        mask = ops.conv_gather(uus[1], P["conv1_t.weight"], P.get("conv1_t.bias"), B, T, ch[1], Fk[0], ch[0], Fk[0], KT=1, S=1, pad=1,
                               act=1, prec=prec)
    else:
        mask = ops.conv_scatter2(u, P["conv1_t.weight"], P["conv1_t.bias"], B, T, ch[1], Fk[1], ch[0], KT=1, pad=0, act=1,
                                 prec=prec)
    _flush_counters()
    if save:
        ctx.update(ys=ys, es=es, stats=stats, gctx=gctx, us=us, vs=vs, dstats=dstats, mask=mask, uus=uus, dec_mode=dec_mode)
        if e_bf is not None and e_bf.dtype == torch.bfloat16:
            ctx["e_bf"] = e_bf.view(B, T, ch[L], Fk[L])
    return mask.view(B, ch[0], T, F0), ctx


def bucket_of(name: str) -> int:
    if name.startswith("gru.gru_list1.") or name.startswith("gru.ln1."):
        return 1
    if name.startswith("gru.") or name.startswith("skip_connect_") or "_t." in name:
        return 0
    return 2


N_BUCKETS = 3


def unet2_backward(ctx, dlogit: torch.Tensor, P: Dict[str, torch.Tensor], G: Dict[str, torch.Tensor],
                   boundary=None, need_dx: bool = False):
    B, T, Fk, ch, L, training = ctx["B"], ctx["T"], ctx["F"], ctx["ch"], ctx["L"], ctx["training"]
    prec = ctx["prec"]
    dprec = prec
    if ops.prec_code(prec) == ops.PREC_BF16:
        dprec = ops.PREC_BF16
    rows = B * T
    ys, es, stats, us, vs, dstats = ctx["ys"], ctx["es"], ctx["stats"], ctx["us"], ctx["vs"], ctx["dstats"]
    _INLINE = config.get().inline_mask
    all_mfma = all(8 <= c <= 64 and (c & (c - 1)) == 0 for c in ch[1:]) and all(ch[k] * Fk[k] <= 640 for k in range(1, L + 1))
    dy_bf16 = bool(config.get().bf16_dy) and ops.prec_code(prec) == ops.PREC_BF16 and dprec == ops.PREC_BF16 and all_mfma
    ups = ctx.get("dec_mode", "transposed") == "upsample"
    uus = ctx.get("uus", {})

    def dec_wgrad(k, dv_):
        if ups and ch[k - 1] % 4 != 0:
            tmp = torch.zeros(ch[k], ch[k - 1], 1, 3, device=dlogit.device, dtype=torch.float32)
            ops.conv_wgrad(uus[k], dv_, tmp, B, T, ch[k], Fk[k - 1], ch[k - 1], Fk[k - 1], KT=1, S=1, pad=1, prec=prec)
            G[f"conv{k}_t.weight"].add_(tmp.flip(-1).permute(1, 0, 2, 3))
        elif ups:
            ops.conv_wgrad(dv_, uus[k], G[f"conv{k}_t.weight"], B, T, ch[k - 1], Fk[k - 1], ch[k], Fk[k - 1], KT=1, S=1, pad=1, prec=prec)
        else:
            ops.conv_wgrad(us[k], dv_, G[f"conv{k}_t.weight"], B, T, ch[k], Fk[k], ch[k - 1], Fk[k - 1], KT=1, S=2, pad=0, prec=prec)

    def dec_dgrad(k, dv_, bn_bwd, out_bf16=False):
        if ups:
            duu = ops.conv_gather(dv_, P[f"conv{k}_t.weight"], None, B, T, ch[k - 1], Fk[k - 1], ch[k], Fk[k - 1], KT=1, S=1, pad=1,
                                  w_layout=1, prec=dprec)
            return ops.downsum_w(duu, rows * ch[k], Fk[k], 2).view(B, T, ch[k], Fk[k]), None
        return split(ops.conv_gather(dv_, P[f"conv{k}_t.weight"], None, B, T, ch[k - 1], Fk[k - 1], ch[k], Fk[k], KT=1, S=2, pad=0,
                                     prec=dprec, bn_bwd=bn_bwd, out_bf16=out_bf16))
    dv = dlogit

    def leaf_dec1(dv=dv):
        if "conv1_t.bias" in G:
            ops.channel_sum(dv, rows, ch[0], Fk[0], G["conv1_t.bias"])
        dec_wgrad(1, dv)
    SIDE.defer(leaf_dec1, dv, kind=2, lane=0)
    fuse_bwd = config.get().fuse_bn_bwd_stats

    def bn_of(k, dec):
        if not fuse_bwd:
            return None
        mean_, rstd_ = dstats[k] if dec else stats[k]
        nm = f"bn{k}_t" if dec else f"bn{k}"
        return ((vs[k] if dec else ys[k]), mean_, rstd_, P[nm + ".weight"], P[nm + ".bias"], True)

    def split(r):
        return r if isinstance(r, tuple) else (r, None)
    de_bf16 = dy_bf16 and bool(config.get().bf16_de) and fuse_bwd and not ups

    def lvl_bf16(k):
        return de_bf16 and 2 <= k < L
    du, du_sums = dec_dgrad(1, dv, bn_of(2, True) if L >= 2 else None)
    ds = {1: du}
    de_pre = {}

    def skip_leaves(k):
        de_pre[k] = torch.empty(B, T, ch[k], Fk[k], device=dlogit.device, dtype=torch.bfloat16 if lvl_bf16(k) else torch.float32)

        def dgrad(k=k, dsk=ds[k], out=de_pre[k]):
            ops.conv_gather(dsk, P[f"skip_connect_{k}.weight"], None, B, T, ch[k], Fk[k], ch[k], Fk[k], KT=1, S=1, pad=1,
                            w_layout=1, out=out, prec=dprec)

        def wgrad(k=k, dsk=ds[k]):
            ek = es[k]
            if k == L and "e_bf" in ctx and ops.prec_code(prec) == ops.PREC_BF16 and all_mfma:
                ek = ctx["e_bf"]
            ops.conv_wgrad(dsk, ek, G[f"skip_connect_{k}.weight"], B, T, ch[k], Fk[k], ch[k], Fk[k], KT=1, S=1, pad=1,
                           prec=prec)
        if _INLINE & 1:
            dgrad()
        else:
            SIDE.defer(dgrad, ds[k], de_pre[k], kind=8, lane=1)
        if _INLINE & 2:
            wgrad()
        else:
            SIDE.defer(wgrad, ds[k], kind=8, lane=1)
    skip_leaves(1)
    fuse_apply = bool(config.get().fuse_bn_bwd_apply) and dy_bf16 and fuse_bwd and not ups
    for k in range(2, L + 1):
        mean, rstd = dstats[k]
        fused = fuse_apply and du.dtype == torch.bfloat16 and du_sums is not None
        if fused:
            du, du_sums, dv = ops.conv_gather_bwd_in(
                du, (vs[k], mean, rstd, P[f"bn{k}_t.weight"], P[f"bn{k}_t.bias"], du_sums, True, training, G[f"bn{k}_t.weight"],
                     G[f"bn{k}_t.bias"], G.get(f"conv{k}_t.bias")),
                P[f"conv{k}_t.weight"], B, T, ch[k - 1], Fk[k - 1], ch[k], Fk[k], KT=1, S=2, pad=0, prec=dprec,
                bn_bwd=bn_of(k + 1, True) if k < L else None, out_bf16=lvl_bf16(k))
        else:
            dv = ops.bn_act_bwd(du, vs[k], mean, rstd, P[f"bn{k}_t.weight"], P[f"bn{k}_t.bias"], rows, ch[k - 1],
                                Fk[k - 1], True, training, G[f"bn{k}_t.weight"], G[f"bn{k}_t.bias"],
                                dbias=G.get(f"conv{k}_t.bias"), sums=du_sums, out_bf16=dy_bf16)

        def leaf_dec(dv=dv, k=k):
            dec_wgrad(k, dv)
        if _INLINE & 4:
            leaf_dec()
        else:
            SIDE.defer(leaf_dec, dv, kind=2, lane=0)
        if not fused:
            du, du_sums = dec_dgrad(k, dv, bn_of(k + 1, True) if k < L else None, out_bf16=lvl_bf16(k))
        ds[k] = du
        skip_leaves(k)
    H = ch[L] * Fk[L]
    marks = {}
    SIDE.after_release = lambda: marks.__setitem__("ev", SIDE.mark())

    def de_pre_ready():
        SIDE.after_release = None
        SIDE.wait(marks["ev"] if "ev" in marks else SIDE.mark())
    de = ggru_backward(ctx["gctx"], du.view(B, T, H), P, G, join=False, dx_init=de_pre[L].view(B, T, H),
                       dx_ready=de_pre_ready, defer_last=boundary is not None).view(B, T, ch[L], Fk[L])
    if boundary is not None:
        boundary(0)
    cut = max(L // 2, 1)
    de_sums = None
    for k in range(L, 0, -1):
        mean, rstd = stats[k]
        fused = fuse_apply and k > 1 and de.dtype == torch.bfloat16 and de_sums is not None
        if fused:
            de_new, de_sums_new, dy = ops.conv_scatter2_bwd_in(
                de, (ys[k], mean, rstd, P[f"bn{k}.weight"], P[f"bn{k}.bias"], de_sums, True, training, G[f"bn{k}.weight"], G[f"bn{k}.bias"],
                     G[f"conv{k}.bias"]),
                P[f"conv{k}.weight"], B, T, ch[k], Fk[k], ch[k - 1], KT=2, pad=1, out=de_pre[k - 1], accum=True, prec=dprec,
                bn_bwd=bn_of(k - 1, False))
        else:
            dy = ops.bn_act_bwd(de, ys[k], mean, rstd, P[f"bn{k}.weight"], P[f"bn{k}.bias"], rows, ch[k], Fk[k], True,
                                training, G[f"bn{k}.weight"], G[f"bn{k}.bias"], dbias=G[f"conv{k}.bias"], sums=de_sums,
                                out_bf16=dy_bf16 and not (need_dx and k == 1))

        def leaf_enc(dy=dy, k=k):
            ops.conv_wgrad(dy, es[k - 1], G[f"conv{k}.weight"], B, T, ch[k], Fk[k], ch[k - 1], Fk[k - 1], KT=2, S=2, pad=1, prec=prec)
        if _INLINE & (8 << (k - 1)):
            leaf_enc()
        else:
            SIDE.run(leaf_enc, dy, lane=0)
        if fused:
            de, de_sums = de_new, de_sums_new
        elif k > 1:
            de, de_sums = split(ops.conv_scatter2(dy, P[f"conv{k}.weight"], None, B, T, ch[k], Fk[k], ch[k - 1], KT=2, pad=1,
                                                  out=de_pre[k - 1], accum=True, prec=dprec, bn_bwd=bn_of(k - 1, False)))
        if boundary is not None and k == cut + 1:
            boundary(1)
    dx = None
    if need_dx:
        dx = ops.conv_scatter2(dy, P["conv1.weight"], None, B, T, ch[1], Fk[1], ch[0], KT=2, pad=1, prec=dprec)
    SIDE.join()
    return dx


class _GGRUFn(torch.autograd.Function):
    @staticmethod
    def forward(ctx, x, mod, names, *params):
        P = dict(zip(names, params))
        need = any(p.requires_grad for p in params) or x.requires_grad
        out, c = ggru_forward(x, P, "", mod.groups, mod.precision, save=need)
        ctx.c, ctx.P, ctx.names = c, P, names
        ctx.need_dx = x.requires_grad
        return out

    @staticmethod
    def backward(ctx, dout):
        P = ctx.P
        G = {n: torch.zeros_like(P[n]) for n in ctx.names}
        dx = ggru_backward(ctx.c, dout.contiguous(), P, G, need_dx=ctx.need_dx)
        return (dx, None, None) + tuple(G[n] for n in ctx.names)


class GGRU(nn.Module):

    def __init__(self, in_features=None, out_features=None, mid_features=None, hidden_size=1024, groups=2,
                 precision: str = DEFAULT_PREC):
        super().__init__()
        hidden_size_t = hidden_size // groups
        self.gru_list1 = nn.ModuleList([nn.GRU(hidden_size_t, hidden_size_t, 1, batch_first=True) for _ in range(groups)])
        self.gru_list2 = nn.ModuleList([nn.GRU(hidden_size_t, hidden_size_t, 1, batch_first=True) for _ in range(groups)])
        self.ln1 = nn.LayerNorm(hidden_size)
        self.ln2 = nn.LayerNorm(hidden_size)
        self.groups = groups
        self.mid_features = mid_features
        self.hidden_size = hidden_size
        self.precision = precision

    def forward(self, x):
        if x.dim() != 4:
            raise RuntimeError(f"GGRU expects [B,C,T,F], got {tuple(x.shape)}")
        B, C, T, F = x.shape
        if C * F != self.hidden_size:
            raise RuntimeError(f"GGRU: C*F = {C * F} does not match hidden_size = {self.hidden_size}")
        rows = x.transpose(1, 2).contiguous().view(B, T, C * F)
        names = [n for n, _ in self.named_parameters()]
        params = [p for _, p in self.named_parameters()]
        out = _GGRUFn.apply(rows, self, names, *params)
        return out.view(B, T, C, F).transpose(1, 2).contiguous()


class _Unet2Fn(torch.autograd.Function):
    @staticmethod
    def forward(ctx, x, mod, names, *params):
        P = dict(zip(names, params))
        Bf = dict(mod.named_buffers())
        need = any(p.requires_grad for p in params)
        mask, c = unet2_forward(x, P, Bf, mod.ch, mod.rnn_groups, mod.precision, mod.training, save=need)
        ctx.c, ctx.P, ctx.names = c, P, names
        return mask

    @staticmethod
    def backward(ctx, dmask):
        P, c = ctx.P, ctx.c
        used = [n for n in ctx.names if not (n.startswith("fc.") or n.startswith("bn1_t."))]
        G = {n: torch.zeros_like(P[n]) for n in used}
        B, T, F0 = c["B"], c["T"], c["F"][0]
        dlogit = ops.sigmoid_bwd(dmask.contiguous().view(B, T, 1, F0), c["mask"])
        unet2_backward(c, dlogit, P, G)
        return (None, None, None) + tuple(G.get(n) for n in ctx.names)


class unet_2(nn.Module):

    def __init__(self, in_feat=161, ch=(1, 8, 16, 32, 64), stride=(1, 2), rnn_groups=4,
                 precision: str = DEFAULT_PREC):
        super().__init__()
        if tuple(stride) != (1, 2):
            raise RuntimeError("cruse_amd unet_2 implements stride (1,2) only (model/cruse_net.py:130 default)")
        self.laynum = len(ch) - 1
        hidden_size = in_feat // 2 ** self.laynum * ch[-1]
        self.ker_x = 2
        self.stride = stride
        self.padding = [self.ker_x - stride[0], 3 - stride[1]]
        for i in range(len(ch) - 1):
            k = i + 1
            setattr(self, f"conv{k}", nn.Conv2d(ch[k - 1], ch[k], (self.ker_x, 3), self.stride, self.padding))
            setattr(self, f"conv{k}_t", nn.ConvTranspose2d(ch[k], ch[k - 1], (1, 3), self.stride))
            setattr(self, f"bn{k}", nn.BatchNorm2d(ch[k]))
            setattr(self, f"bn{k}_t", nn.BatchNorm2d(ch[k - 1]))
            setattr(self, f"skip_connect_{k}", nn.Conv2d(ch[k], ch[k], (1, 3), padding=(0, 1), bias=False))
        self.gru = GGRU(hidden_size=hidden_size, groups=rnn_groups, precision=precision)
        self.elu = nn.ReLU()
        self.fc = nn.Linear(in_feat, in_feat)
        self.ch = tuple(ch)
        self.rnn_groups = rnn_groups
        self.in_feat = in_feat
        self.hidden_size = hidden_size
        self.precision = precision

    def set_precision(self, precision: str) -> None:
        self.precision = precision
        self.gru.precision = precision

    def forward(self, x):
        if x.shape[-1] * self.ch[-1] // (1 << self.laynum) != self.hidden_size:
            raise RuntimeError(f"unet_2: {x.shape[-1]} input bins give hidden size "
                               f"{x.shape[-1] * self.ch[-1] // (1 << self.laynum)}, expected {self.hidden_size}")
        names = [n for n, _ in self.named_parameters()]
        params = [p for _, p in self.named_parameters()]
        return _Unet2Fn.apply(x.contiguous(), self, names, *params)
```

cruse_amd/ops.py:

```python
from __future__ import annotations

import ctypes
from typing import Dict, List, Optional, Sequence

import torch

from ._lib import PREC_BF16, PREC_BF16X3, PREC_BY_NAME, PREC_F32, check, lib


def _stream() -> int:
    return torch.cuda.current_stream().cuda_stream


def _p(t: Optional[torch.Tensor]):
    if t is None:
        return None
    if not t.is_cuda:
        raise RuntimeError("cruse_amd ops need tensors on the HIP device (no CPU fallback)")
    if not t.is_contiguous():
        raise RuntimeError(f"cruse_amd ops need contiguous tensors, got strides {t.stride()} for shape {tuple(t.shape)}")
    return t.data_ptr()


def _xdt(t: torch.Tensor, name: str) -> int:
# ... 187 lines not shown

def _conv_bnin(scatter, bn, w, bias, B, T, Cin, Fin, Cout, Fout, KT, S, pad, prec, publish, copy_bf16, want_sums, out):
    if out is None:
        out = _conv_out(w, B, T, Cout, Fout)
    sums, z = _bn_sums(Cout, w.device) if want_sums else _NO_SUMS
    check(_CONV_FN[scatter][3](*bn.args(publish, copy_bf16), _p(w), _p(bias), _p(out), *_geom(scatter, B, T, Cin, Fin, Cout, Fout, KT, S, pad),
                               conv_prec(prec), _p(sums), z, _stream()))
    return (out, sums) if want_sums else out


def conv_gather_bnin(bn: BnIn, w, bias, B, T, Cin, Fin, Cout, Fout, KT, S, pad, prec, publish=False, copy_bf16=None, want_sums=False,
                     out=None):
    return _conv_bnin(False, bn, w, bias, B, T, Cin, Fin, Cout, Fout, KT, S, pad, prec, publish, copy_bf16, want_sums, out)


def conv_scatter2_bnin(bn: BnIn, w, bias, B, T, Cs, Fg, Cout, KT, pad, prec, publish=False, copy_bf16=None, want_sums=False):
    return _conv_bnin(True, bn, w, bias, B, T, Cs, Fg, Cout, 2 * Fg, KT, 2, pad, prec, publish, copy_bf16, want_sums, None)


def _conv_bnstats(scatter, x, w, bias, B, T, Cin, Fin, Cout, Fout, KT, S, pad, prec):
    out = _conv_out(x, B, T, Cout, Fout)
    sums, z = _bn_sums(Cout, x.device)
    check(_CONV_FN[scatter][4](_p(x), _p(w), _p(bias), _p(out), *_geom(scatter, B, T, Cin, Fin, Cout, Fout, KT, S, pad), conv_prec(prec),
                               _p(sums), z, _stream()))
    return out, sums


def conv_gather_bnstats(x, w, bias, B, T, Cin, Fin, Cout, Fout, KT, S, pad, prec=None):
    return _conv_bnstats(False, x, w, bias, B, T, Cin, Fin, Cout, Fout, KT, S, pad, prec)


def conv_scatter2_bnstats(g, w, bias, B, T, Cs, Fg, Cout, KT, pad, prec=None):
    return _conv_bnstats(True, g, w, bias, B, T, Cs, Fg, Cout, 2 * Fg, KT, 2, pad, prec)


def conv_plan(scatter, Cin, Fin, Cout, Fout, KT, S, pad, w_layout, B, T, prec, x_dtype=0, y_dtype=0, act=0, accum=0, forms=0) -> dict:
    out = (ctypes.c_int * 7)()
    check(lib.cruse_conv_plan(1 if scatter else 0, Cin, Fin, Cout, Fout, KT, S, pad, w_layout, B, T, conv_prec(prec), x_dtype, y_dtype, act,
                              1 if accum else 0, forms, ctypes.cast(out, ctypes.c_void_p)))
    return {"route": "mfma" if out[0] else "valu", "fused": bool(out[1]), "mt": out[2], "nw": out[3], "grid": out[4], "lds_bytes": out[5],
            "co_t": out[6]}


_wgrad_ws = {}
_ws_retired = []


def _ws(key, nbytes: int, device, zero: bool = True) -> torch.Tensor:
    device = torch.device(device)
    if device.type == "cuda" and device.index is None:
        device = torch.device("cuda", torch.cuda.current_device())
    buf = _wgrad_ws.get((key, device))
    if buf is None or buf.numel() < nbytes:
        old = buf
        buf = (torch.zeros if zero else torch.empty)(nbytes, dtype=torch.uint8, device=device)
        if old is not None:
            _ws_retired.append((key, old))
        _wgrad_ws[(key, device)] = buf
    return buf


_gru_hdr: Dict[torch.device, torch.Tensor] = {}


def gru_header(device) -> torch.Tensor:
    device = torch.device(device)
    if device.type == "cuda" and device.index is None:
        device = torch.device("cuda", torch.cuda.current_device())
    h = _gru_hdr.get(device)
    if h is None:
        h = _gru_hdr[device] = torch.zeros(256, dtype=torch.uint8, device=device)
    return h


WGRAD_PREC = {"f32": PREC_F32, "bf16x3": PREC_BF16X3, "bf16": PREC_BF16, "valu": -1}


def conv_wgrad(a, bt, dw, B, T, Ca, Fa, Cb, Fb, KT, S, pad, prec=None):
    nbytes = lib.cruse_conv_wgrad_ws_bytes(Ca, Cb, KT)
    ws = _ws(("wgrad", _stream()), nbytes, a.device, zero=False)
    pc = -1 if prec is None else (WGRAD_PREC[prec] if isinstance(prec, str) else int(prec))
    check(lib.cruse_conv_wgrad(_p(a), _p(bt), _p(dw), B, T, Ca, Fa, Cb, Fb, KT, S, pad, pc, _xdt(a, "conv_wgrad a"),
                               _xdt(bt, "conv_wgrad bt"), _p(ws), _stream()))


def upsample_w(x, rows, W, up=2):
    _f32(x, "upsample_w")
    out = torch.empty(rows, W * up, device=x.device, dtype=torch.float32)
    check(lib.cruse_upsample_w(_p(x), rows, W, up, _p(out), 0, _stream()))
    return out


def downsum_w(dxu, rows, W, up=2):
    _f32(dxu, "downsum_w")
    out = torch.empty(rows, W, device=dxu.device, dtype=torch.float32)
    check(lib.cruse_downsum_w(_p(dxu), rows, W, up, _p(out), 0, _stream()))
    return out


def channel_sum(g, rows, C, F, out):
    check(lib.cruse_channel_sum(_p(g), rows, C, F, _p(out), _stream()))


def col_sum(g, g_off, rows, ncol, ld, out):
    check(lib.cruse_col_sum(g.data_ptr() + 4 * g_off, rows, ncol, ld, _p(out), _stream()))


class _ZeroArena:

    CAP = 1 << 14

    def __init__(self):
        self.bufs = {}
        self.active = None
        self.off = 0

    def step(self, device):
        arena = self

        class _Ctx:
            def __enter__(self_):
                dev = torch.device(device)
                buf = arena.bufs.get(dev)
                if buf is None:
                    buf = arena.bufs[dev] = torch.zeros(arena.CAP, device=dev, dtype=torch.float64)
                arena.active, arena.off = buf, 0
                zero_(buf)
                return arena

            def __exit__(self_, *exc):
                arena.active = None
        return _Ctx()

    def take(self, n: int, device):
        if self.active is None or self.active.device != device or self.off + n > self.CAP:
            return torch.empty(n, device=device, dtype=torch.float64), 0
        t = self.active[self.off:self.off + n]
        self.off += (n + 1) // 2 * 2
        return t, 1


ARENA = _ZeroArena()


def bn_stats(y, rows, C, F):
    sums, z = ARENA.take(2 * C, y.device)
    check(lib.cruse_bn_stats(_p(y), rows, C, F, _p(sums), z, _stream()))
    return sums


BN_STAT_REPLICAS = 16


def bn_finalize_act_fwd(y, sums, count, eps, momentum, gamma, beta, skip, rows, C, F, relu=True, running_mean=None,
                        running_var=None, out_bf16=None):
    if sums.numel() % (2 * C) != 0:
        raise RuntimeError(f"bn_finalize_act_fwd: {sums.numel()} sums for {C} channels")
    out = torch.empty_like(y)
    mean = torch.empty(C, device=y.device, dtype=torch.float32)
    rstd = torch.empty(C, device=y.device, dtype=torch.float32)
    if out_bf16 is not None and (out_bf16.dtype not in (torch.bfloat16, torch.float16) or out_bf16.numel() < y.numel()):
        raise RuntimeError("bn_finalize_act_fwd: out_bf16 must be a bf16 (or f16) tensor of at least y.numel() elements")
    check(lib.cruse_bn_finalize_act_fwd_c(_p(y), _p(sums), sums.numel() // (2 * C), count, eps, momentum, _p(gamma), _p(beta), _p(skip), _p(out),
                                          _p(out_bf16), _copy_dt(out_bf16), _p(mean), _p(rstd), _p(running_mean), _p(running_var), rows, C, F,
                                          1 if relu else 0, _stream()))
    return out, mean, rstd


def bn_finalize(sums, count, C, eps, momentum, running_mean=None, running_var=None):
    mean = torch.empty(C, device=sums.device, dtype=torch.float32)
    rstd = torch.empty(C, device=sums.device, dtype=torch.float32)
    check(lib.cruse_bn_finalize(_p(sums), count, C, eps, momentum, _p(mean), _p(rstd), _p(running_mean),
                                _p(running_var), _stream()))
    return mean, rstd


def bn_eval_stats(running_mean, running_var, eps):
    C = running_mean.numel()
    mean = torch.empty(C, device=running_mean.device, dtype=torch.float32)
    rstd = torch.empty(C, device=running_mean.device, dtype=torch.float32)
    check(lib.cruse_bn_eval_stats(_p(running_mean), _p(running_var), C, eps, _p(mean), _p(rstd), _stream()))
    return mean, rstd


def bn_act_fwd(y, mean, rstd, gamma, beta, skip, rows, C, F, relu=True):
    out = torch.empty_like(y)
    check(lib.cruse_bn_act_fwd(_p(y), _p(mean), _p(rstd), _p(gamma), _p(beta), _p(skip), _p(out), rows, C, F,
                               1 if relu else 0, _stream()))
    return out


def bn_act_bwd(dout, y, mean, rstd, gamma, beta, rows, C, F, relu, training, dgamma, dbeta, dbias=None, sums=None,
               out_bf16=False):
    nrep = BN_STAT_REPLICAS
    if sums is None:
        nrep = 1
        sums, z = ARENA.take(2 * C, y.device)
        _f32(dout, "bn_act_bwd (reduce pass) dout")
        check(lib.cruse_bn_act_bwd_reduce(_p(dout), _p(y), _p(mean), _p(rstd), _p(gamma), _p(beta), rows, C, F,
                                          1 if relu else 0, _p(sums), z, _stream()))
    dy = torch.empty_like(y, dtype=torch.bfloat16 if out_bf16 else torch.float32)
    check(lib.cruse_bn_act_bwd_apply(_p(dout), _p(y), _p(mean), _p(rstd), _p(gamma), _p(beta), _p(sums), nrep, rows, C, F,
                                     1 if relu else 0, 1 if training else 0, _xdt(dout, "bn_act_bwd dout"), _p(dy), 2 if out_bf16 else 0,
                                     _p(dgamma), _p(dbeta),
                                     _p(dbias), _stream()))
    return dy


def _copy_dt(t) -> int:
    return 1 if (t is not None and t.dtype == torch.float16) else 2


def ln_fwd(x, gamma, beta, res, rows, H, interleave_g=1, eps=1e-5, save=True, out=None, out_bf16=None, seg=None, stats=None):
    y = torch.empty_like(x) if out is None else out
    if stats is not None:
        mean, rstd = stats
    else:
        nstat = x.numel() // H
        mean = torch.empty(nstat, device=x.device, dtype=torch.float32) if save else None
        rstd = torch.empty(nstat, device=x.device, dtype=torch.float32) if save else None
    sl, ss, so = seg if seg is not None else (0, 0, 0)
    if out_bf16 is not None and (out_bf16.dtype not in (torch.bfloat16, torch.float16) or out_bf16.numel() < x.numel()):
        raise RuntimeError("ln_fwd: out_bf16 must be a bf16 (or f16) tensor of at least x.numel() elements")
    check(lib.cruse_ln_fwd_c(_p(x), _p(gamma), _p(beta), _p(res), _p(y), _p(out_bf16), _copy_dt(out_bf16), _p(mean), _p(rstd), rows, H,
                             interleave_g, eps, sl, ss, so, _stream()))
    return y, mean, rstd


def ln_bwd(dy, x, mean, rstd, gamma, rows, H, interleave_g, dgamma, dbeta):
    dx = torch.empty_like(x)
    check(lib.cruse_ln_bwd(_p(dy), _p(x), _p(mean), _p(rstd), _p(gamma), rows, H, interleave_g, _p(dx), _p(dgamma),
                           _p(dbeta), _stream()))
    return dx


def gemm(transA, transB, M, N, K, A, a_off, lda, Bm, b_off, ldb, C, c_off, ldc, bias=None, accumulate=False,
         splitk=1, b_shift_T=0, prec=PREC_F32):
    pa = A.data_ptr() + 4 * a_off
    pb = Bm.data_ptr() + 4 * b_off
    pc = C.data_ptr() + 4 * c_off
    check(lib.cruse_gemm(1 if transA else 0, 1 if transB else 0, M, N, K, pa, lda, pb, ldb, pc, ldc, _p(bias),
                         1 if accumulate else 0, splitk, b_shift_T, prec_code(prec), _stream()))


def gemm_bf16_nt(M, N, K, A, a_off, lda, Bm, b_off, ldb, C, c_off, ldc, bias=None, accumulate=False, splitk=1,
                 a_kstride=64, b_kstride=64, slabs=False):
    if slabs and accumulate and bias is None and abs(splitk) > 1 and N % 4 == 0 and C.dtype == torch.float32:
        if A.dtype != torch.bfloat16 or Bm.dtype != torch.bfloat16:
            raise RuntimeError("gemm_bf16_nt needs bf16 operands")
        nbytes = lib.cruse_gemm_bf16_slab_bytes(M, N, splitk)
        ws = _ws(("gemm_slabs", _stream()), nbytes, C.device, zero=False)
        check(lib.cruse_gemm_bf16_nt_slabs(M, N, K, A.data_ptr() + 2 * a_off, lda, a_kstride, Bm.data_ptr() + 2 * b_off, ldb, b_kstride,
                                           C.data_ptr() + 4 * c_off, ldc, splitk, _p(ws), ws.numel(), _stream()))
        return
    if C.dtype in _OUT16 and A.dtype == torch.bfloat16 and Bm.dtype == torch.bfloat16 and not accumulate and abs(splitk) <= 1:
        return _gemm_nt_out16(M, N, K, A, None, a_off, lda, a_kstride, Bm, None, b_off, ldb, b_kstride, C, c_off, ldc, bias, False)
    if A.dtype != torch.bfloat16 or Bm.dtype != torch.bfloat16 or C.dtype != torch.float32:
        raise RuntimeError("gemm_bf16_nt needs bf16 operands and an f32 result")
    check(lib.cruse_gemm_bf16_nt(M, N, K, A.data_ptr() + 2 * a_off, lda, a_kstride, Bm.data_ptr() + 2 * b_off, ldb, b_kstride,
                                 C.data_ptr() + 4 * c_off, ldc, _p(bias), 1 if accumulate else 0, splitk, _stream()))


def gemm_bf16_nt_cat(Ms, N, K, A, a_rows, lda, Bs, b_off, ldb, C, c_off, ldc, splitk, a_kstride=64, b_kstride=64):
    n = len(Ms)
    if A.dtype != torch.bfloat16 or any(b.dtype != torch.bfloat16 for b in Bs) or C.dtype != torch.float32:
        raise RuntimeError("gemm_bf16_nt_cat needs bf16 operands and an f32 result")
    nbytes = lib.cruse_gemm_bf16_slab_bytes(int(sum(Ms)), N, splitk)
    ws = _ws(("gemm_slabs", _stream()), nbytes, C.device, zero=False)
    ms = (ctypes.c_int * n)(*[int(m) for m in Ms])
    ar = (ctypes.c_longlong * n)(*[int(r) for r in a_rows])
    bs = (ctypes.c_void_p * n)(*[b.data_ptr() + 2 * b_off for b in Bs])
    check(lib.cruse_gemm_bf16_nt_slabs_cat(n, ctypes.cast(ms, ctypes.c_void_p), N, K, A.data_ptr(), ctypes.cast(ar, ctypes.c_void_p), lda, a_kstride,
                                           ctypes.cast(bs, ctypes.c_void_p), ldb, b_kstride, C.data_ptr() + 4 * c_off, ldc, splitk, _p(ws),
                                           ws.numel(), _stream()))


def gemm_bf16_nt_atr(M, N, K, A_T, a_off, a_mb_stride, n_mb, Bm, b_off, ldb, C, c_off, ldc, accumulate=False, b_kstride=64):
    if A_T.dtype != torch.bfloat16 or Bm.dtype != torch.bfloat16 or C.dtype != torch.float32:
        raise RuntimeError("gemm_bf16_nt_atr needs bf16 operands and an f32 result")
    check(lib.cruse_gemm_bf16_nt_atr(M, N, K, A_T.data_ptr() + 2 * a_off, a_mb_stride, n_mb, Bm.data_ptr() + 2 * b_off, ldb, b_kstride,
                                     C.data_ptr() + 4 * c_off, ldc, 1 if accumulate else 0, _stream()))
    return C


def gemm_bf16_nt_groups(M, N, K, G, A_hi, A_lo, lda, a_gstep, B_hi, B_lo, ldb, b_gstep, C, ldc, c_gstep, bias=None, bias_gstep=0,
                        accumulate=False, b_kstride=64):
    for t_ in (A_hi, A_lo, B_hi, B_lo):
        if t_ is not None and t_.dtype != torch.bfloat16:
            raise RuntimeError("gemm_bf16_nt_groups needs bf16 planes")
    if C.dtype != torch.float32:
        raise RuntimeError("gemm_bf16_nt_groups: f32 result")
    check(lib.cruse_gemm_bf16_nt_groups(M, N, K, G, _p(A_hi), _p(A_lo), lda, a_gstep, _p(B_hi), _p(B_lo), ldb, b_kstride, b_gstep,
                                        _p(C), ldc, c_gstep, _p(bias), bias_gstep, 1 if accumulate else 0, _stream()))
    return C


def uniform_stride(tensors) -> Optional[int]:
    if len(tensors) < 2:
        return 0
    d = [tensors[i + 1].data_ptr() - tensors[i].data_ptr() for i in range(len(tensors) - 1)]
    if any(x != d[0] for x in d) or d[0] <= 0 or d[0] % 4:
        return None
    return d[0] // 4


def gemm_bf16_nt_seg(M, N, K, A_hi, A_lo, a_off, lda, B_hi, B_lo, b_off, ldb, C, c_off, ldc, seg, bias=None, accumulate=False,
                     b_kstride=64):
    lo = lambda t_, off: None if t_ is None else t_.data_ptr() + 2 * off
    check(lib.cruse_gemm_bf16_nt_seg(M, N, K, A_hi.data_ptr() + 2 * a_off, lo(A_lo, a_off), lda, B_hi.data_ptr() + 2 * b_off,
                                     lo(B_lo, b_off), ldb, b_kstride, C.data_ptr() + 4 * c_off, ldc, _p(bias),
                                     1 if accumulate else 0, seg[0], seg[1], seg[2], _stream()))


def cast_bf16(x, out=None):
    y = torch.empty(x.shape, device=x.device, dtype=torch.bfloat16) if out is None else out
    check(lib.cruse_cast_bf16(_p(x), _p(y), x.numel(), _stream()))
    return y


def ktile_bf16(x, rows, cols, split=False, out=None):
    if out is not None:
        y, lo = out
    else:
        y = torch.empty((cols + 63) // 64, rows, 64, device=x.device, dtype=torch.bfloat16)
        lo = torch.empty_like(y) if split else None
    check(lib.cruse_ktile_bf16(_p(x), rows, cols, cols, _p(y), _p(lo), _stream()))
    return (y, lo) if split else y


def ktile_f16(x, rows, cols, split=False):
    y = torch.empty((cols + 63) // 64, rows, 64, device=x.device, dtype=torch.float16)
    if split:
        lo = torch.empty_like(y)
        check(lib.cruse_ktile_f16_split(_p(x), rows, cols, cols, _p(y), _p(lo), _stream()))
        return y, lo
    check(lib.cruse_ktile_f16(_p(x), rows, cols, cols, _p(y), _stream()))
    return y


_OUT16 = {torch.float16: 1, torch.bfloat16: 2}


def _gemm_nt_out16(M, N, K, A_hi, A_lo, a_off, lda, a_kstride, B_hi, B_lo, b_off, ldb, b_kstride, C, c_off, ldc, bias, operands_f16):
    check(lib.cruse_gemm_nt_out16(M, N, K, A_hi.data_ptr() + 2 * a_off, None if A_lo is None else A_lo.data_ptr() + 2 * a_off, lda, a_kstride,
                                  B_hi.data_ptr() + 2 * b_off, None if B_lo is None else B_lo.data_ptr() + 2 * b_off, ldb, b_kstride,
                                  C.data_ptr() + 2 * c_off, ldc, _p(bias), 1 if operands_f16 else 0, _OUT16[C.dtype], _stream()))
    return C


def gemm_f16_nt(M, N, K, A, a_off, lda, B, b_off, ldb, C, c_off, ldc, bias=None, a_kstride=64, b_kstride=64, B_lo=None):
    if A.dtype != torch.float16 or B.dtype != torch.float16 or (B_lo is not None and B_lo.dtype != torch.float16):
        raise RuntimeError("gemm_f16_nt needs f16 operands")
    if C.dtype in _OUT16:
        return _gemm_nt_out16(M, N, K, A, None, a_off, lda, a_kstride, B, B_lo, b_off, ldb, b_kstride, C, c_off, ldc, bias, True)
    if C.dtype != torch.float32:
        raise RuntimeError("gemm_f16_nt: the result is f32, or f16 / bf16 rows (cruse_gemm_nt_out16)")
    if B_lo is not None:
        check(lib.cruse_gemm_f16x2_nt(M, N, K, A.data_ptr() + 2 * a_off, lda, a_kstride, B.data_ptr() + 2 * b_off, B_lo.data_ptr() + 2 * b_off, ldb,
# ... 770 lines not shown
```

include/cruse_hip.h:

```cpp
#ifndef CRUSE_HIP_H
#define CRUSE_HIP_H

#include <stddef.h>

#ifdef __cplusplus
extern "C" {
#endif

#define CRUSE_ABI_VERSION 14

enum {
    CRUSE_OK = 0,
    CRUSE_E_SHAPE = -1,
    CRUSE_E_ALIGN = -2,
    CRUSE_E_DTYPE = -3,
    CRUSE_E_HIP = -4,
    CRUSE_E_TIMEOUT = -5
};

enum {
    CRUSE_PREC_F32 = 0,
    CRUSE_PREC_BF16X3 = 1,
    CRUSE_PREC_BF16 = 2,
    CRUSE_PREC_F16 = 3
};

enum {
    CRUSE_DT_F32 = 0,
    CRUSE_DT_F16 = 1,
    CRUSE_DT_BF16 = 2
};

int cruse_abi_version(void);
const char* cruse_last_error(void);
int cruse_set_option(const char* name, int value, int unset);
int cruse_get_option(const char* name, int* value, int* is_set);


int cruse_stft_fwd(const float* wave, int B, int L, int n_fft, int hop,
                   float* re, float* im, float* mag, int mag_bins, float mag_eps, void* stream);

int cruse_istft_fwd(const float* re, const float* im, int B, int T, int n_fft, int hop, int L,
                    float* wave, void* stream);
int cruse_istft_bwd(const float* dwave, int B, int T, int n_fft, int hop, int L,
                    float* dre, float* dim, void* stream);


int cruse_conv_gather(const float* x, const float* w, const float* bias, float* y,
                      int B, int T, int Cin, int Fin, int Cout, int Fout,
                      int KT, int S, int pad, int w_layout, int act, int accum, int prec, int x_dtype, int y_dtype, void* stream);

int cruse_conv_scatter2(const float* g, const float* w, const float* bias, float* y,
                        int B, int T, int Cs, int Fg, int Cout, int Fout,
                        int KT, int pad, int act, int accum, int prec, int x_dtype, int y_dtype, void* stream);

#define CRUSE_BN_STAT_REPLICAS 16
int cruse_conv_gather_bnstats(const float* x, const float* w, const float* bias, float* y,
                              int B, int T, int Cin, int Fin, int Cout, int Fout,
                              int KT, int S, int pad, int prec, double* sums, int zeroed, void* stream);
int cruse_conv_scatter2_bnstats(const float* g, const float* w, const float* bias, float* y,
                                int B, int T, int Cs, int Fg, int Cout, int Fout,
                                int KT, int pad, int prec, double* sums, int zeroed, void* stream);

int cruse_conv_gather_bnin(const float* x_pre, const double* in_sums, int in_replicas, long long in_count, float eps, float momentum,
                           const float* in_gamma, const float* in_beta, float* in_mean, float* in_rstd, float* in_running_mean,
                           float* in_running_var, const float* in_add, void* in_copy_bf16,
                           const float* w, const float* bias, float* y, int B, int T, int Cin, int Fin, int Cout, int Fout,
                           int KT, int S, int pad, int prec, double* out_sums, int zeroed, void* stream);
int cruse_conv_scatter2_bnin(const float* g_pre, const double* in_sums, int in_replicas, long long in_count, float eps, float momentum,
                             const float* in_gamma, const float* in_beta, float* in_mean, float* in_rstd, float* in_running_mean,
                             float* in_running_var, const float* in_add, void* in_copy_bf16,
                             const float* w, const float* bias, float* y, int B, int T, int Cs, int Fg, int Cout, int Fout,
                             int KT, int pad, int prec, double* out_sums, int zeroed, void* stream);

int cruse_conv_gather_bnbwd(const float* x, const float* w, float* y, int B, int T, int Cin, int Fin, int Cout, int Fout,
                            int KT, int S, int pad, int w_layout, int accum, int prec,
                            const float* bn_y, const float* mean, const float* rstd, const float* gamma, const float* beta,
                            int relu, double* sums, int zeroed, int x_dtype, int y_dtype, void* stream);
int cruse_conv_scatter2_bnbwd(const float* g, const float* w, float* y, int B, int T, int Cs, int Fg, int Cout, int Fout,
                              int KT, int pad, int accum, int prec,
                              const float* bn_y, const float* mean, const float* rstd, const float* gamma, const float* beta,
                              int relu, double* sums, int zeroed, int x_dtype, int y_dtype, void* stream);

int cruse_conv_gather_bnbwd_in(const void* dout, int dout_dtype, const float* in_y, const float* in_mean, const float* in_rstd,
                               const float* in_gamma, const float* in_beta, const double* in_sums, int in_replicas, int in_relu,
                               int in_training, void* dy_bf16, float* in_dgamma, float* in_dbeta, float* in_dbias,
                               const float* w, void* y, int B, int T, int Cin, int Fin, int Cout, int Fout, int KT, int S, int pad,
                               int w_layout, int accum, int prec,
                               const float* bn_y, const float* mean, const float* rstd, const float* gamma, const float* beta, int relu,
                               double* sums, int zeroed, int y_dtype, void* stream);
int cruse_conv_scatter2_bnbwd_in(const void* dout, int dout_dtype, const float* in_y, const float* in_mean, const float* in_rstd,
                                 const float* in_gamma, const float* in_beta, const double* in_sums, int in_replicas, int in_relu,
                                 int in_training, void* dy_bf16, float* in_dgamma, float* in_dbeta, float* in_dbias,
                                 const float* w, void* y, int B, int T, int Cs, int Fg, int Cout, int Fout, int KT, int pad, int accum,
                                 int prec,
                                 const float* bn_y, const float* mean, const float* rstd, const float* gamma, const float* beta, int relu,
                                 double* sums, int zeroed, int y_dtype, void* stream);

int cruse_conv_mfma_stamps(unsigned long long* out8);

enum { CRUSE_CONV_FORM_SUMS = 1, CRUSE_CONV_FORM_BNB = 2, CRUSE_CONV_FORM_BNI = 4, CRUSE_CONV_FORM_BBI = 8 };
int cruse_conv_plan(int scatter, int Cin, int Fin, int Cout, int Fout, int KT, int S, int pad, int w_layout,
                    int B, int T, int prec, int x_dtype, int y_dtype, int act, int accum, int forms, int* out);

size_t cruse_conv_wgrad_ws_bytes(int Ca, int Cb, int KT);
int cruse_conv_wgrad(const float* a, const float* bt, float* dw,
                     int B, int T, int Ca, int Fa, int Cb, int Fb,
                     int KT, int S, int pad, int prec, int a_dtype, int bt_dtype, void* ws, void* stream);

int cruse_channel_sum(const float* g, long long rows, int C, int F, float* out, void* stream);
int cruse_col_sum(const float* g, long long rows, int ncol, int ld, float* out, void* stream);


int cruse_bn_stats(const float* y, long long rows, int C, int F, double* sums, int zeroed, void* stream);
int cruse_bn_finalize(const double* sums, long long count, int C, float eps, float momentum,
                      float* mean, float* rstd, float* running_mean, float* running_var, void* stream);
int cruse_bn_eval_stats(const float* running_mean, const float* running_var, int C, float eps,
                        float* mean, float* rstd, void* stream);
int cruse_bn_act_fwd(const float* y, const float* mean, const float* rstd, const float* gamma,
                     const float* beta, const float* skip, float* out,
                     long long rows, int C, int F, int relu, void* stream);
int cruse_bn_finalize_act_fwd(const float* y, const double* sums, int sum_replicas, long long count, float eps, float momentum,
                              const float* gamma, const float* beta, const float* skip, float* out, void* out_bf16,
                              float* mean, float* rstd, float* running_mean, float* running_var,
                              long long rows, int C, int F, int relu, void* stream);
int cruse_bn_finalize_act_fwd_c(const float* y, const double* sums, int sum_replicas, long long count, float eps, float momentum,
                                const float* gamma, const float* beta, const float* skip, float* out, void* out_copy, int copy_dtype,
                                float* mean, float* rstd, float* running_mean, float* running_var,
                                long long rows, int C, int F, int relu, void* stream);
int cruse_bn_act_bwd_reduce(const float* dout, const float* y, const float* mean, const float* rstd,
                            const float* gamma, const float* beta, long long rows, int C, int F,
                            int relu, double* sums, int zeroed, void* stream);
int cruse_bn_act_bwd_apply(const float* dout, const float* y, const float* mean, const float* rstd,
                           const float* gamma, const float* beta, const double* sums, int sum_replicas,
                           long long rows, int C, int F, int relu, int training, int dout_dtype,
                           void* dy, int dy_dtype, float* dgamma, float* dbeta, float* dbias, void* stream);


int cruse_ln_fwd(const float* x, const float* gamma, const float* beta, const float* res,
                 float* y, void* y_bf16, float* mean, float* rstd, long long rows, int H, int interleave_g,
                 float eps, int seg_len, long long seg_stride, long long seg_off, void* stream);
int cruse_ln_fwd_c(const float* x, const float* gamma, const float* beta, const float* res,
                   float* y, void* y_copy, int copy_dtype, float* mean, float* rstd, long long rows, int H, int interleave_g,
                   float eps, int seg_len, long long seg_stride, long long seg_off, void* stream);
int cruse_ln_bwd(const float* dy, const float* x, const float* mean, const float* rstd,
                 const float* gamma, long long rows, int H, int interleave_g,
                 float* dx, float* dgamma, float* dbeta, void* stream);


int cruse_gemm(int transA, int transB, int M, int N, int K,
               const float* A, int lda, const float* B, int ldb, float* C, int ldc,
               const float* bias, int accumulate, int splitk, int b_shift_T, int prec, void* stream);

int cruse_gemm_bf16_nt(int M, int N, int K, const void* A, long long lda, long long a_kstride,
                       const void* B, long long ldb, long long b_kstride,
                       float* C, long long ldc, const float* bias, int accumulate, int splitk, void* stream);
size_t cruse_gemm_bf16_slab_bytes(int M, int N, int splitk);
int cruse_gemm_bf16_nt_slabs(int M, int N, int K, const void* A, long long lda, long long a_kstride,
                             const void* B, long long ldb, long long b_kstride,
                             float* C, long long ldc, int splitk, void* scratch, size_t scratch_bytes, void* stream);
int cruse_gemm_bf16_nt_slabs_cat(int nprob, const int* Ms, int N, int K, const void* A, const long long* a_rows, long long lda,
                                 long long a_kstride, const void* const* Bs, long long ldb, long long b_kstride,
                                 float* C, long long ldc, int splitk, void* scratch, size_t scratch_bytes, void* stream);
int cruse_gemm_bf16_nt_groups(int M, int N, int K, int G, const void* A_hi, const void* A_lo, long long lda, long long a_gstep,
                              const void* B_hi, const void* B_lo, long long ldb, long long b_kstride, long long b_gstep,
                              float* C, long long ldc, long long c_gstep, const float* bias, long long bias_gstep, int accumulate,
                              void* stream);
int cruse_gemm_bf16_nt_seg(int M, int N, int K, const void* A_hi, const void* A_lo, long long lda,
                           const void* B_hi, const void* B_lo, long long ldb, long long b_kstride,
                           float* C, long long ldc, const float* bias, int accumulate,
                           int seg_len, long long seg_stride, long long seg_off, void* stream);
int cruse_cast_bf16(const float* x, void* y, long long n, void* stream);
int cruse_ktile_bf16(const float* x, int rows, int cols, long long ld, void* y, void* y_lo, void* stream);
int cruse_ktile_f16(const float* x, int rows, int cols, long long ld, void* y, void* stream);
int cruse_ktile_f16_split(const float* x, int rows, int cols, long long ld, void* y, void* y_lo, void* stream);
int cruse_gemm_bf16_nt_atr(int M, int N, int K, const void* A_T, long long a_mb_stride, int n_mb,
                           const void* B, long long ldb, long long b_kstride,
                           float* C, long long ldc, int accumulate, void* stream);
int cruse_gemm_nt_out16(int M, int N, int K, const void* A_hi, const void* A_lo, long long lda, long long a_kstride,
                        const void* B_hi, const void* B_lo, long long ldb, long long b_kstride,
                        void* C, long long ldc, const float* bias, int operands_f16, int out_dtype, void* stream);
int cruse_gemm_f16_nt(int M, int N, int K, const void* A, long long lda, long long a_kstride,
                      const void* B, long long ldb, long long b_kstride,
                      float* C, long long ldc, const float* bias, void* stream);
int cruse_gemm_f16x2_nt(int M, int N, int K, const void* A, long long lda, long long a_kstride,
                        const void* B_hi, const void* B_lo, long long ldb, long long b_kstride,
                        float* C, long long ldc, const float* bias, void* stream);
int cruse_cast_bf16_split(const float* x, void* y, void* y_lo, long long n, void* stream);
int cruse_gemm_bf16x3_nt(int M, int N, int K, const void* A_hi, const void* A_lo, long long lda, long long a_kstride,
                         const void* B_hi, const void* B_lo, long long ldb, long long b_kstride,
                         float* C, long long ldc, const float* bias, int accumulate, void* stream);
int cruse_transpose_bf16(const float* x, long long rows, int cols, long long ld, void* yT, long long ldT,
                         int shift_T, void* stream);


size_t cruse_gru_ws_bytes(int B, int G, int Hg);
int cruse_gru_plan(int B, int G, int Hg, int prec, int fwd, int* out);
int cruse_gru_seq_fwd(const float* gi, const float* const* w_hh, const float* const* b_hh,
                      float* h, void* coef, float* an, float* z,
                      int B, int T, int G, int Hg, int prec, void* ws, void* stream);
int cruse_gru_seq_bwd(const float* dout, const float* const* w_hh, const void* coef, const float* z,
                      float* dh, int B, int T, int G, int Hg, int prec, void* ws, void* stream);
int cruse_gru_seq_fwd_on(const float* gi, const float* const* w_hh, const float* const* b_hh,
                         float* h, void* coef, float* an, float* z,
                         int B, int T, int G, int Hg, int prec, void* panels, unsigned* status, int xcd_rot, void* stream);
int cruse_gru_seq_bwd_on(const float* dout, const float* const* w_hh, const void* coef, const float* z,
                         float* dh, const float* an, void* dgi, int B, int T, int G, int Hg, int prec,
                         void* panels, unsigned* status, int xcd_rot, void* stream);
int cruse_gru_seq_fwd_ex(const float* gi, const float* const* w_hh, const float* const* b_hh,
                         float* h, void* coef, float* an, float* z, const float* h0, long long h0_bstride,
                         int B, int T, int TS, int G, int Hg, int prec, int chain_clips, void* panels,
                         int panels_zeroed, unsigned* status, int xcd_rot, void* stream);
int cruse_gru_seq_bwd_ex(const float* dout, const float* const* w_hh, const void* coef, const float* z,
                         float* dh, const float* an, void* dgi, int dg_slabs, int carry, int B, int T, int TS, int G,
                         int Hg, int prec, int chain_clips, void* panels, int panels_zeroed, unsigned* status, int xcd_rot,
                         void* stream);
int cruse_gru_seq_fwd_gi16(const void* gi, int gi_dtype, const float* const* w_hh, const float* const* b_hh,
                           float* h, void* coef, float* an, float* z,
                           int B, int T, int TS, int G, int Hg, int prec, void* panels,
                           int panels_zeroed, unsigned* status, int xcd_rot, void* stream);
int cruse_gru_gate_grads(const float* dh, const void* coef, const float* an, float* dgi, float* dgh,
                         long long rows, int G, int Hg, int prec, void* stream);
int cruse_gru_gate_grads_bf16(const float* dh, const void* coef, const float* an, void* dgi, void* dgT,
                              long long ldT, float* const* db_ih, float* const* db_hh,
                              long long rows, int G, int Hg, void* stream);


int cruse_mask_loss_fwd(const float* mask, const float* nre, const float* nim, const float* cmag,
                        long long rows, int Fn, int Fs, float alpha, float beta,
                        double* loss_sum, float* dmask, float* dlogit, float* est_re, float* est_im,
                        void* stream);


int cruse_mask_apply(const float* mask, const float* nre, const float* nim, long long rows, int Fn, int Fs,
                     float* est_re, float* est_im, void* stream);
int cruse_mask_apply_bwd(const float* dre, const float* dim, const float* nre, const float* nim,
                         const float* mask, long long rows, int Fn, int Fs, int through_sigmoid,
                         float* dout, void* stream);
int cruse_mask_sdnr_fwd(const float* mask, const float* cre, const float* cim, const float* nre, const float* nim,
                        long long rows, int Fn, int Fs, int B, float snr_db, float beta_db,
                        double* loss_sum, float* dmask, float* dlogit, void* stream);
int cruse_sisnr_fwd(const float* x, const float* s, int B, int L, float eps,
                    double* mom, double* loss, float* coef, void* stream);
int cruse_sisnr_bwd(const float* x, const float* s, const float* coef, int B, int L, float grad_scale,
                    float* dx, void* stream);
int cruse_wave_l1_mse(const float* est, const float* ref, long long n, int mse, float grad_scale,
                      double* loss_sum, float* dest, void* stream);

int cruse_deepfilter_fwd(const float* xr, const float* xi, const float* hr, const float* hi,
                         int B, int F, int T, int f_dim, int t_dim, float* out_r, float* out_i, void* stream);
int cruse_deepfilter_bwd(const float* dout_r, const float* dout_i, const float* xr, const float* xi,
                         const float* hr, const float* hi, int B, int F, int T, int f_dim, int t_dim,
                         float* dxr, float* dxi, float* dhr, float* dhi, void* stream);

int cruse_sigmoid_bwd(const float* dmask, const float* mask, float* dlogit, long long n, void* stream);

int cruse_axpby(float* out, const float* x, const float* y, float a, float b, long long n, void* stream);


int cruse_conv2d_nchw(const void* x, const float* w, const float* bias, void* y,
                      int B, int Cin, int Hin, int Win, int Cout, int Hout, int Wout,
                      int KH, int KW, int sh, int sw, int dh, int dw, int pt, int pl,
                      int groups, int up_w, int transposed, int act, const float* slope, int accumulate, int dtype,
                      void* stream);
int cruse_conv2d_nchw_wgrad(const void* S, const void* Bg, float* dw,
                            int N, int CA, int HS, int WS, int CB, int HB, int WB,
                            int KH, int KW, int sh, int sw, int dh, int dw_, int pt, int pl,
                            int groups, int up_w, int dtype, void* stream);
int cruse_conv2d_nchw_wgrad_ex(const void* S, const void* Bg, float* dw, float* db,
                               int N, int CA, int HS, int WS, int CB, int HB, int WB,
                               int KH, int KW, int sh, int sw, int dh, int dw_, int pt, int pl,
                               int groups, int up_w, int dtype, void* stream);
int cruse_nchw_channel_sum(const void* x, int N, int C, int HW, float* out, int dtype, void* stream);
int cruse_downsum_w(const void* dxu, long long rows, int W, int up, void* dx, int dtype, void* stream);
int cruse_upsample_w(const void* x, long long rows, int W, int up, void* xu, int dtype, void* stream);
int cruse_bn_nchw_stats(const void* x, int N, int C, int HW, double* sums, int dtype, void* stream);
int cruse_bn_nchw_fwd(const void* x, const float* mean, const float* rstd, const float* gamma, const float* beta,
                      const float* slope, int act, int N, int C, int HW, void* y, int dtype, void* stream);
int cruse_bn_nchw_bwd(const void* dy, const void* x, const float* mean, const float* rstd, const float* gamma,
                      const float* beta, const float* slope, int act, int training, int N, int C, int HW,
                      double* scratch, void* dx, float* dgamma, float* dbeta, float* dslope, int dtype, void* stream);

int cruse_bn_nchw_fwd_train(const void* x, const double* sums, int sum_replicas, float eps, float momentum, const float* gamma, const float* beta,
                            const float* slope, int act, int N, int C, int HW, void* y, float* mean_out, float* rstd_out,
                            float* running_mean, float* running_var, long long* num_batches_tracked, int dtype, void* stream);
int cruse_conv2d_nchw_ex(const void* x, const float* w, const float* bias, const void* residual, void* y,
                         int B, int Cin, int Hin, int Win, int Cout, int Hout, int Wout,
                         int KH, int KW, int sh, int sw, int dh, int dw, int pt, int pl,
                         int groups, int up_w, int transposed, int act, const float* slope,
// ... 149 lines not shown
```

Before: 5.497 million.

## Save packed f16 normalized activations with ReLU mask for BatchNorm backward

Result: no change. 5.518 million (median of 6 runs) (+0.4%).

```diff
diff --git a/cruse_amd/_lib.py b/cruse_amd/_lib.py
--- a/cruse_amd/_lib.py
+++ b/cruse_amd/_lib.py
@@ -46,6 +46,9 @@
     "cruse_bn_act_fwd": ("pppppppqiiip", "i"),
     "cruse_bn_act_bwd_reduce": ("ppppppqiiipip", "i"),
     "cruse_bn_act_bwd_apply": ("pppppppiqiiiiipipppp", "i"),
+    "cruse_bn_finalize_act_fwd_x16": ("ppiqffpppppipppppqiiip", "i"),
+    "cruse_bn_act_bwd_reduce_x16": ("ppqiiipip", "i"),
+    "cruse_bn_act_bwd_apply_x16": ("pppppiqiiiiipipppp", "i"),
     "cruse_ln_fwd": ("ppppppppqiifiqqp", "i"),
     "cruse_ln_fwd_c": ("ppppppippqiifiqqp", "i"),
     "cruse_ln_bwd": ("pppppqiipppp", "i"),
diff --git a/cruse_amd/config.py b/cruse_amd/config.py
--- a/cruse_amd/config.py
+++ b/cruse_amd/config.py
@@ -21,6 +21,7 @@
     bf16_de: bool = True
     gi_store_f16: bool = False
     dx_atr: bool = True
+    bn_bwd_copy16: bool = True
     pick_launch_stream: bool = True
     lib_options: Dict[str, int] = field(default_factory=dict)
 
@@ -32,7 +33,7 @@
              
             "fuse_bn_fwd": ("CRUSE_FUSE_BN_FWD", lambda v: v != "0"), "fuse_bn_bwd_apply": ("CRUSE_FUSE_BN_BWD_APPLY", lambda v: v != "0"), "bf16_dy": ("CRUSE_BF16_DY", lambda v: v != "0"), "bf16_de": ("CRUSE_BF16_DE", lambda v: v != "0"),
             "pick_launch_stream": ("CRUSE_PICK_LAUNCH_STREAM", lambda v: v != "0"), "gi_store_f16": ("CRUSE_GI_STORE_F16", lambda v: v != "0"),
-            "dx_atr": ("CRUSE_DX_ATR", lambda v: v != "0")}
+            "dx_atr": ("CRUSE_DX_ATR", lambda v: v != "0"), "bn_bwd_copy16": ("CRUSE_BN_BWD_COPY16", lambda v: v != "0")}
     _LIB_ENV = {"CRUSE_GRU_BWD_RS": "gru_bwd_rs", "CRUSE_GRU_FWD_LEAN": "gru_fwd_lean", "CRUSE_GRU_WLO": "gru_wlo", "CRUSE_GRU_DBG": "gru_dbg",
                 "CRUSE_GRU_TF": "gru_tf", "CRUSE_GRU_POLL_FWD": "gru_poll_fwd", "CRUSE_GRU_POLL_BWD": "gru_poll_bwd", "CRUSE_CM_KINT": "cm_kint",
                 "CRUSE_CM_SWAP": "cm_swap", "CRUSE_CM_NW": "cm_nw", "CRUSE_PW_VALU": "pw_valu", "CRUSE_WG_DBG": "wg_dbg",
diff --git a/cruse_amd/csrc/pointwise.hip b/cruse_amd/csrc/pointwise.hip
--- a/cruse_amd/csrc/pointwise.hip
+++ b/cruse_amd/csrc/pointwise.hip
@@ -145,11 +145,26 @@
     }
 }
 
+__device__ __forceinline__ unsigned xh16_pack(const float xh, const bool pass) {
+    unsigned u = __float_as_uint(xh);
+    if ((u & 0x7f800000u) != 0x7f800000u) { u += 0x1fffu + ((u >> 14) & 1u); u &= ~0x3fffu; }
+    const _Float16 h = (_Float16)__uint_as_float(u);
+    return (unsigned)(__builtin_bit_cast(unsigned short, h) & 0xfffeu) | (pass ? 1u : 0u);
+}
+__device__ __forceinline__ float xh16_val(const unsigned w) { return (float)__builtin_bit_cast(_Float16, (unsigned short)(w & 0xfffeu)); }
+__device__ __forceinline__ void xh16_load4(const unsigned short* cp, const long long i, float (&xh)[4], bool (&pass)[4]) {
+    const uint2 w = *reinterpret_cast<const uint2*>(cp + i);
+    const unsigned ww[4] = {w.x & 0xffffu, w.x >> 16, w.y & 0xffffu, w.y >> 16};
+#pragma unroll
+    for (int e = 0; e < 4; ++e) { xh[e] = xh16_val(ww[e]); pass[e] = (ww[e] & 1u) != 0u; }
+}
+
+template <bool X16>
 __global__ __launch_bounds__(256) void bn_fin_act_fwd_kernel(const float* y, const double* sums, int nrep, double inv_count, double unb,
                                                              float eps, float momentum, const float* gamma,
                                                              const float* beta, const float* skip, float* out, __bf16* out_bf,
                                                              float* mean_o, float* rstd_o, float* rmean, float* rvar,
-                                                             long long rows, int C, int F, int relu, int copy_f16) {
+                                                             long long rows, int C, int F, int relu, int copy_f16, unsigned short* xh16) {
     extern __shared__ float tab[];
     for (int c = threadIdx.x; c < C; c += 256) {
         double t1 = 0.0, t2 = 0.0;
@@ -203,14 +218,23 @@
                     const long long i = r * CF + q * 4;
                     const float in[4] = {vv[g].x, vv[g].y, vv[g].z, vv[g].w}, sk[4] = {ss[g].x, ss[g].y, ss[g].z, ss[g].w};
                     float o[4];
+                    unsigned wd[4];
 #pragma unroll
                     for (int e = 0; e < 4; ++e) {
-                        float t = (in[e] - pm[g][e]) * pr[g][e] * pg[g][e] + pb[g][e];
+                        float t;
+                        if constexpr (X16) {
+                            const float xh = (in[e] - pm[g][e]) * pr[g][e];
+                            t = xh * pg[g][e] + pb[g][e];
+                            wd[e] = xh16_pack(xh, !relu || t > 0.f);
+                        } else {
+                            t = (in[e] - pm[g][e]) * pr[g][e] * pg[g][e] + pb[g][e];
+                        }
                         if (relu) t = fmaxf(t, 0.f);
                         o[e] = t + sk[e];
                     }
                     *reinterpret_cast<float4*>(out + i) = make_float4(o[0], o[1], o[2], o[3]);
                     if (out_bf) store_copy4(out_bf, i, o[0], o[1], o[2], o[3], copy_f16);
+                    if constexpr (X16) *reinterpret_cast<uint2*>(xh16 + i) = make_uint2(wd[0] | (wd[1] << 16), wd[2] | (wd[3] << 16));
                 }
             }
         }
@@ -237,52 +261,70 @@
     }
 }
 
-__global__ __launch_bounds__(RED_THREADS) void bn_act_bwd_reduce_kernel(const float* dout, const float* y, const float* mean,
+template <bool X16>
+__global__ __launch_bounds__(RED_THREADS) void bn_act_bwd_reduce_kernel(const float* dout, const void* y_, const float* mean,
                                                                 const float* rstd, const float* gamma,
                                                                 const float* beta, long long rows, int C, int F,
                                                                 int relu, double* sums) {
-    __shared__ float tab[4][256];
+    __shared__ float tab[X16 ? 1 : 4][256];
     float pm[CPR_MAXG][4], pr[CPR_MAXG][4], pg[CPR_MAXG][4], pb[CPR_MAXG][4];
     const int lane = threadIdx.x & 63;
-    for (int c = threadIdx.x; c < C; c += blockDim.x) {
-        tab[0][c] = mean[c]; tab[1][c] = rstd[c]; tab[2][c] = gamma[c]; tab[3][c] = beta[c];
-    }
-    __syncthreads();
-#pragma unroll
-    for (int g = 0; g < CPR_MAXG; ++g)
-#pragma unroll
-        for (int e = 0; e < 4; ++e) {
-            const int col = (lane + 64 * g) * 4 + e;
-            const int c = col < C * F ? col / F : 0;
-            pm[g][e] = tab[0][c]; pr[g][e] = tab[1][c]; pg[g][e] = tab[2][c]; pb[g][e] = tab[3][c];
-        }
+    if constexpr (!X16) {
+        for (int c = threadIdx.x; c < C; c += blockDim.x) {
+            tab[0][c] = mean[c]; tab[1][c] = rstd[c]; tab[2][c] = gamma[c]; tab[3][c] = beta[c];
+        }
+        __syncthreads();
+#pragma unroll
+        for (int g = 0; g < CPR_MAXG; ++g)
+#pragma unroll
+            for (int e = 0; e < 4; ++e) {
+                const int col = (lane + 64 * g) * 4 + e;
+                const int c = col < C * F ? col / F : 0;
+                pm[g][e] = tab[0][c]; pr[g][e] = tab[1][c]; pg[g][e] = tab[2][c]; pb[g][e] = tab[3][c];
+            }
+    }
     channel_pair_reduce(rows, C, F, sums, [&](long long i, int g, float (&v)[4], float (&v2)[4]) {
-        const float4 yy = *reinterpret_cast<const float4*>(y + i);
         const float4 dd = *reinterpret_cast<const float4*>(dout + i);
-        const float yv[4] = {yy.x, yy.y, yy.z, yy.w}, dv[4] = {dd.x, dd.y, dd.z, dd.w};
-#pragma unroll
-        for (int e = 0; e < 4; ++e) {
-            const float xh = (yv[e] - pm[g][e]) * pr[g][e];
-            float gr = dv[e];
-            if (relu && !(xh * pg[g][e] + pb[g][e] > 0.f)) gr = 0.f;
-            v[e] = gr; v2[e] = gr * xh;
+        const float dv[4] = {dd.x, dd.y, dd.z, dd.w};
+        if constexpr (X16) {
+            float xh[4];
+            bool pass[4];
+            xh16_load4(static_cast<const unsigned short*>(y_), i, xh, pass);
+#pragma unroll
+            for (int e = 0; e < 4; ++e) {
+                const float gr = (relu && !pass[e]) ? 0.f : dv[e];
+                v[e] = gr; v2[e] = gr * xh[e];
+            }
+        } else {
+            const float4 yy = *reinterpret_cast<const float4*>(static_cast<const float*>(y_) + i);
+            const float yv[4] = {yy.x, yy.y, yy.z, yy.w};
+#pragma unroll
+            for (int e = 0; e < 4; ++e) {
+                const float xh = (yv[e] - pm[g][e]) * pr[g][e];
+                float gr = dv[e];
+                if (relu && !(xh * pg[g][e] + pb[g][e] > 0.f)) gr = 0.f;
+                v[e] = gr; v2[e] = gr * xh;
+            }
         }
     });
 }
 
-__global__ __launch_bounds__(256) void bn_act_bwd_apply_kernel(const float* dout, const float* y, const float* mean,
+template <bool X16>
+__global__ __launch_bounds__(256) void bn_act_bwd_apply_kernel(const float* dout, const void* y_, const float* mean,
                                                                const float* rstd, const float* gamma,
                                                                const float* beta, const double* sums, int nrep, long long rows,
                                                                int C, int F, int relu, int training, float* dy, int dy_bf16,
                                                                int dout_bf16, float* dgamma, float* dbeta, float* dbias) {
     __shared__ float tab[6][256];
+    const float* const y = static_cast<const float*>(y_);
+    const unsigned short* const yx = static_cast<const unsigned short*>(y_);
     const double cnt = (double)rows * F;
     const int tid = threadIdx.x, lane = tid & 63;
     const int CF = C * F, ng = CF >> 2;
     for (int c = tid; c < C; c += 256) {
         double sg = 0.0, sgx = 0.0;
         for (int r = 0; r < nrep; ++r) { sg += sums[(size_t)r * 2 * C + c]; sgx += sums[(size_t)r * 2 * C + C + c]; }
-        tab[0][c] = mean[c]; tab[1][c] = rstd[c]; tab[2][c] = gamma[c]; tab[3][c] = beta[c];
+        tab[0][c] = X16 ? 0.f : mean[c]; tab[1][c] = rstd[c]; tab[2][c] = gamma[c]; tab[3][c] = X16 ? 0.f : beta[c];
         tab[4][c] = training ? (float)(sg / cnt) : 0.f;
         tab[5][c] = training ? (float)(sgx / cnt) : 0.f;
         if (blockIdx.x == 0) {
@@ -304,14 +346,15 @@
         }
     const long long wave = (long long)blockIdx.x * 4 + (tid >> 6), nwave = (long long)gridDim.x * 4;
     for (long long r = wave; r < rows; r += nwave) {
-        float4 vv[CPR_MAXG], dv[CPR_MAXG];
+        float4 vv[X16 ? 1 : CPR_MAXG], dv[CPR_MAXG];
+        uint2 vx[X16 ? CPR_MAXG : 1];
         if (dout_bf16) {
 #pragma unroll
             for (int g = 0; g < CPR_MAXG; ++g) {
                 const int q = lane + 64 * g;
                 if (q < ng) {
                     const long long i = r * CF + q * 4;
-                    vv[g] = *reinterpret_cast<const float4*>(y + i);
+                    if constexpr (X16) vx[g] = *reinterpret_cast<const uint2*>(yx + i); else vv[g] = *reinterpret_cast<const float4*>(y + i);
                     const float2 w2 = *reinterpret_cast<const float2*>(reinterpret_cast<const __bf16*>(dout) + i);
                     const unsigned w0 = __float_as_uint(w2.x), w1 = __float_as_uint(w2.y);
                     dv[g] = make_float4(__uint_as_float(w0 << 16), __uint_as_float(w0 & 0xffff0000u), __uint_as_float(w1 << 16),
@@ -324,7 +367,7 @@
                 const int q = lane + 64 * g;
                 if (q < ng) {
                     const long long i = r * CF + q * 4;
-                    vv[g] = *reinterpret_cast<const float4*>(y + i);
+                    if constexpr (X16) vx[g] = *reinterpret_cast<const uint2*>(yx + i); else vv[g] = *reinterpret_cast<const float4*>(y + i);
                     dv[g] = *reinterpret_cast<const float4*>(dout + i);
                 }
             }
@@ -334,14 +377,25 @@
             const int q = lane + 64 * g;
             if (q < ng) {
                 const long long i = r * CF + q * 4;
-                const float in[4] = {vv[g].x, vv[g].y, vv[g].z, vv[g].w}, dd[4] = {dv[g].x, dv[g].y, dv[g].z, dv[g].w};
+                const float dd[4] = {dv[g].x, dv[g].y, dv[g].z, dv[g].w};
                 float o[4];
-#pragma unroll
-                for (int e = 0; e < 4; ++e) {
-                    const float xh = (in[e] - pm[g][e]) * pr[g][e];
-                    float gr = dd[e];
-                    if (relu && !(xh * pg[g][e] + pb[g][e] > 0.f)) gr = 0.f;
-                    o[e] = pg[g][e] * pr[g][e] * (gr - p1[g][e] - xh * p2[g][e]);
+                if constexpr (X16) {
+                    const unsigned ww[4] = {vx[g].x & 0xffffu, vx[g].x >> 16, vx[g].y & 0xffffu, vx[g].y >> 16};
+#pragma unroll
+                    for (int e = 0; e < 4; ++e) {
+                        const float xh = xh16_val(ww[e]);
+                        const float gr = (relu && !(ww[e] & 1u)) ? 0.f : dd[e];
+                        o[e] = pg[g][e] * pr[g][e] * (gr - p1[g][e] - xh * p2[g][e]);
+                    }
+                } else {
+                    const float in[4] = {vv[g].x, vv[g].y, vv[g].z, vv[g].w};
+#pragma unroll
+                    for (int e = 0; e < 4; ++e) {
+                        const float xh = (in[e] - pm[g][e]) * pr[g][e];
+                        float gr = dd[e];
+                        if (relu && !(xh * pg[g][e] + pb[g][e] > 0.f)) gr = 0.f;
+                        o[e] = pg[g][e] * pr[g][e] * (gr - p1[g][e] - xh * p2[g][e]);
+                    }
                 }
                 if (dy_bf16) {
                     typedef __attribute__((ext_vector_type(4))) __bf16 bf16x4_;
@@ -809,6 +863,11 @@
                                            float* mean, float* rstd, float* running_mean, float* running_var,
                                            long long rows, int C, int F, int relu, void* stream);
 
+extern "C" int cruse_bn_finalize_act_fwd_x16(const float* y, const double* sums, int sum_replicas, long long count, float eps, float momentum,
+                                             const float* gamma, const float* beta, const float* skip, float* out, void* out_copy, int copy_dtype,
+                                             void* xh16, float* mean, float* rstd, float* running_mean, float* running_var,
+                                             long long rows, int C, int F, int relu, void* stream);
+
 extern "C" int cruse_bn_finalize_act_fwd(const float* y, const double* sums, int sum_replicas, long long count, float eps, float momentum,
                                          const float* gamma, const float* beta, const float* skip, float* out, void* out_bf16,
                                          float* mean, float* rstd, float* running_mean, float* running_var,
@@ -821,15 +880,24 @@
                                            const float* gamma, const float* beta, const float* skip, float* out, void* out_bf16, int copy_dtype,
                                            float* mean, float* rstd, float* running_mean, float* running_var,
                                            long long rows, int C, int F, int relu, void* stream) {
+    return cruse_bn_finalize_act_fwd_x16(y, sums, sum_replicas, count, eps, momentum, gamma, beta, skip, out, out_bf16, copy_dtype, nullptr, mean, rstd,
+                                         running_mean, running_var, rows, C, F, relu, stream);
+}
+
+extern "C" int cruse_bn_finalize_act_fwd_x16(const float* y, const double* sums, int sum_replicas, long long count, float eps, float momentum,
+                                             const float* gamma, const float* beta, const float* skip, float* out, void* out_bf16, int copy_dtype,
+                                             void* xh16, float* mean, float* rstd, float* running_mean, float* running_var,
+                                             long long rows, int C, int F, int relu, void* stream) {
     CRUSE_REQUIRE(copy_dtype == CRUSE_DT_BF16 || copy_dtype == CRUSE_DT_F16, CRUSE_E_DTYPE, "bn_finalize_act_fwd: copy_dtype %d (bf16 or f16)", copy_dtype);
     CRUSE_REQUIRE(rows > 0 && C > 0 && C <= 256 && F > 0 && count > 0 && sum_replicas >= 1, CRUSE_E_SHAPE, "bn_finalize_act_fwd: bad shape");
     CRUSE_REQUIRE((C * F) % 4 == 0, CRUSE_E_ALIGN, "bn_finalize_act_fwd: C*F=%d must be a multiple of 4", C * F);
     CRUSE_REQUIRE((running_mean == nullptr) == (running_var == nullptr) && mean && rstd, CRUSE_E_SHAPE, "bn_finalize_act_fwd: statistics");
     const double unb = count > 1 ? (double)count / (double)(count - 1) : 1.0;
     const bool rowwise = C * F <= 64 * CPR_MAXG * 4 && (C * F) % 4 == 0;
-    hipLaunchKernelGGL(bn_fin_act_fwd_kernel, dim3(rowwise ? grid_for(rows, 8, 2048) : grid_for(rows * C * F / 4, 1024)), dim3(256), 4 * C * sizeof(float), ST(stream),
+    CRUSE_REQUIRE(xh16 == nullptr || rowwise, CRUSE_E_SHAPE, "bn_finalize_act_fwd_x16: the backward copy needs C*F=%d <= %d", C * F, 64 * CPR_MAXG * 4);
+    hipLaunchKernelGGL(xh16 ? bn_fin_act_fwd_kernel<true> : bn_fin_act_fwd_kernel<false>, dim3(rowwise ? grid_for(rows, 8, 2048) : grid_for(rows * C * F / 4, 1024)), dim3(256), 4 * C * sizeof(float), ST(stream),
                        y, sums, sum_replicas, 1.0 / (double)count, unb, eps, momentum, gamma, beta, skip, out, (__bf16*)out_bf16, mean, rstd, running_mean,
-                       running_var, rows, C, F, relu, copy_dtype == CRUSE_DT_F16 ? 1 : 0);
+                       running_var, rows, C, F, relu, copy_dtype == CRUSE_DT_F16 ? 1 : 0, static_cast<unsigned short*>(xh16));
     CRUSE_LAUNCH_CHECK("bn_finalize_act_fwd");
     return CRUSE_OK;
 }
@@ -840,9 +908,21 @@
     CRUSE_REQUIRE(rows > 0 && C > 0 && C <= 256 && F > 0, CRUSE_E_SHAPE, "bn_act_bwd_reduce: bad shape");
     CRUSE_REQUIRE((C * F) % 4 == 0 && C * F <= 768, CRUSE_E_SHAPE, "bn_act_bwd_reduce: C*F=%d must be a multiple of 4 and <= 768", C * F);
     if (!zeroed) { int zrc = cruse_zero_async(sums, 2 * C * sizeof(double), ST(stream), "bn_act_bwd_reduce memset"); if (zrc) return zrc; }
-    hipLaunchKernelGGL(bn_act_bwd_reduce_kernel, dim3(grid_for(rows, 64, 256)), dim3(RED_THREADS), 0, ST(stream), dout, y, mean,
+    hipLaunchKernelGGL(bn_act_bwd_reduce_kernel<false>, dim3(grid_for(rows, 64, 256)), dim3(RED_THREADS), 0, ST(stream), dout, (const void*)y, mean,
                        rstd, gamma, beta, rows, C, F, relu, sums);
     CRUSE_LAUNCH_CHECK("bn_act_bwd_reduce");
+    return CRUSE_OK;
+}
+
+extern "C" int cruse_bn_act_bwd_reduce_x16(const float* dout, const void* xh16, long long rows, int C, int F, int relu, double* sums, int zeroed,
+                                           void* stream) {
+    CRUSE_REQUIRE(dout && xh16 && sums, CRUSE_E_SHAPE, "bn_act_bwd_reduce_x16: NULL tensor");
+    CRUSE_REQUIRE(rows > 0 && C > 0 && C <= 256 && F > 0, CRUSE_E_SHAPE, "bn_act_bwd_reduce_x16: bad shape");
+    CRUSE_REQUIRE((C * F) % 4 == 0 && C * F <= 768, CRUSE_E_SHAPE, "bn_act_bwd_reduce_x16: C*F=%d must be a multiple of 4 and <= 768", C * F);
+    if (!zeroed) { int zrc = cruse_zero_async(sums, 2 * C * sizeof(double), ST(stream), "bn_act_bwd_reduce_x16 memset"); if (zrc) return zrc; }
+    hipLaunchKernelGGL(bn_act_bwd_reduce_kernel<true>, dim3(grid_for(rows, 64, 256)), dim3(RED_THREADS), 0, ST(stream), dout, xh16, (const float*)nullptr,
+                       (const float*)nullptr, (const float*)nullptr, (const float*)nullptr, rows, C, F, relu, sums);
+    CRUSE_LAUNCH_CHECK("bn_act_bwd_reduce_x16");
     return CRUSE_OK;
 }
 
@@ -855,10 +935,26 @@
     CRUSE_REQUIRE(rows > 0 && C > 0 && C <= 256 && F > 0 && sum_replicas >= 1, CRUSE_E_SHAPE, "bn_act_bwd_apply: bad shape");
     CRUSE_REQUIRE((C * F) % 4 == 0 && C * F <= 768, CRUSE_E_SHAPE,
                   "bn_act_bwd_apply: C*F=%d must be a multiple of 4 and <= 768", C * F);
-    hipLaunchKernelGGL(bn_act_bwd_apply_kernel, dim3(grid_for(rows, 8, 2048)), dim3(256), 0, ST(stream), dout, y,
+    hipLaunchKernelGGL(bn_act_bwd_apply_kernel<false>, dim3(grid_for(rows, 8, 2048)), dim3(256), 0, ST(stream), dout, (const void*)y,
                        mean, rstd, gamma, beta, sums, sum_replicas, rows, C, F, relu, training, (float*)dy,
                        dy_dtype == CRUSE_DT_BF16 ? 1 : 0, dout_dtype == CRUSE_DT_BF16 ? 1 : 0, dgamma, dbeta, dbias);
     CRUSE_LAUNCH_CHECK("bn_act_bwd_apply");
+    return CRUSE_OK;
+}
+
+extern "C" int cruse_bn_act_bwd_apply_x16(const void* dout, const void* xh16, const float* rstd, const float* gamma, const double* sums,
+                                          int sum_replicas, long long rows, int C, int F, int relu, int training, int dout_dtype,
+                                          void* dy, int dy_dtype, float* dgamma, float* dbeta, float* dbias, void* stream) {
+    CRUSE_REQUIRE((dy_dtype == CRUSE_DT_F32 || dy_dtype == CRUSE_DT_BF16) && (dout_dtype == CRUSE_DT_F32 || dout_dtype == CRUSE_DT_BF16),
+                  CRUSE_E_DTYPE, "bn_act_bwd_apply_x16: dout_dtype %d / dy_dtype %d (f32 or bf16)", dout_dtype, dy_dtype);
+    CRUSE_REQUIRE(dout && xh16 && rstd && gamma && sums && dy, CRUSE_E_SHAPE, "bn_act_bwd_apply_x16: NULL tensor");
+    CRUSE_REQUIRE(rows > 0 && C > 0 && C <= 256 && F > 0 && sum_replicas >= 1, CRUSE_E_SHAPE, "bn_act_bwd_apply_x16: bad shape");
+    CRUSE_REQUIRE((C * F) % 4 == 0 && C * F <= 768, CRUSE_E_SHAPE,
+                  "bn_act_bwd_apply_x16: C*F=%d must be a multiple of 4 and <= 768", C * F);
+    hipLaunchKernelGGL(bn_act_bwd_apply_kernel<true>, dim3(grid_for(rows, 8, 2048)), dim3(256), 0, ST(stream), static_cast<const float*>(dout), xh16,
+                       (const float*)nullptr, rstd, gamma, (const float*)nullptr, sums, sum_replicas, rows, C, F, relu, training, (float*)dy,
+                       dy_dtype == CRUSE_DT_BF16 ? 1 : 0, dout_dtype == CRUSE_DT_BF16 ? 1 : 0, dgamma, dbeta, dbias);
+    CRUSE_LAUNCH_CHECK("bn_act_bwd_apply_x16");
     return CRUSE_OK;
 }
 
diff --git a/cruse_amd/model/cruse_net.py b/cruse_amd/model/cruse_net.py
--- a/cruse_amd/model/cruse_net.py
+++ b/cruse_amd/model/cruse_net.py
@@ -516,7 +516,7 @@
         _PENDING_COUNTERS.clear()
 
 
-def _bn_act(y, rows, C, F, P, Bf, name, training, update_running, skip=None, sums=None, out_bf16=None):
+def _bn_act(y, rows, C, F, P, Bf, name, training, update_running, skip=None, sums=None, out_bf16=None, xh16=None):
     gamma, beta = P[name + ".weight"], P[name + ".bias"]
     if training:
         if sums is None:
@@ -526,7 +526,7 @@
         if update_running:
             _PENDING_COUNTERS.append(Bf[name + ".num_batches_tracked"])
         return ops.bn_finalize_act_fwd(y, sums, rows * F, BN_EPS, BN_MOMENTUM, gamma, beta, skip, rows, C, F, relu=True,
-                                       running_mean=rm, running_var=rv, out_bf16=out_bf16)
+                                       running_mean=rm, running_var=rv, out_bf16=out_bf16, xh16=xh16)
     mean, rstd = ops.bn_eval_stats(Bf[name + ".running_mean"], Bf[name + ".running_var"], BN_EPS)
     return ops.bn_act_fwd(y, mean, rstd, gamma, beta, skip, rows, C, F, relu=True), mean, rstd
 
@@ -553,6 +553,14 @@
     fz = (training and save and config.get().fuse_bn_fwd and config.get().fuse_bn_stats
           and all(ch[k] * Fk[k] <= 640 for k in range(1, L + 1)))
     dev = x.device
+    cp16 = training and save and bool(config.get().bn_bwd_copy16) and ops.prec_code(prec) == ops.PREC_BF16
+    xh = {}
+
+    def backward_copy(name, C, F):
+        if not (cp16 and ops.xh16_eligible(C, F)):
+            return None
+        xh[name] = torch.empty(B, T, C, F, device=dev, dtype=torch.int16)
+        return xh[name]
 
     def virtual(y_, sums_, C, F, name, add=None):
         mean_ = torch.empty(C, device=dev, dtype=torch.float32); rstd_ = torch.empty(C, device=dev, dtype=torch.float32)
@@ -590,7 +598,10 @@
             if k == L and training and _gi_takes_bf16_copy(prec, ch[L] * Fk[L] // groups):
                 e_bf = torch.empty(rows * ch[L] * Fk[L], device=x.device,
                                    dtype=torch.float16 if _gi_f16(prec, ch[L] * Fk[L] // groups, 0) else torch.bfloat16)
-            e, mean, rstd = _bn_act(y, rows, ch[k], Fk[k], P, Bf, f"bn{k}", training, update_running, sums=sums, out_bf16=e_bf)
+            e, mean, rstd = _bn_act(y, rows, ch[k], Fk[k], P, Bf, f"bn{k}", training, update_running, sums=sums, out_bf16=e_bf,
+                                    xh16=backward_copy(f"bn{k}", ch[k], Fk[k]) if k == L else None)
+            if f"bn{k}" in xh:
+                y = None
 
             def skip_conv(e=e, s=s, k=k):
                 ops.conv_gather(e, P[f"skip_connect_{k}.weight"], None, B, T, ch[k], Fk[k], ch[k], Fk[k], KT=1, S=1, pad=1,
@@ -632,8 +643,12 @@
             mean, rstd = pend.mean, pend.rstd
         else:
             pend = None
+            dec1_valu = k == 2 and not ups and ops.conv_plan(False, ch[0], Fk[0], ch[1], Fk[1], 1, 2, 0, 0, B, T, ops.PREC_BF16,
+                                                             forms=ops.CONV_FORM_BNB)["route"] == "valu"
             u, mean, rstd = _bn_act(v, rows, ch[k - 1], Fk[k - 1], P, Bf, f"bn{k}_t", training, update_running, skip=ss[k - 1],
-                                    sums=sums)
+                                    sums=sums, xh16=backward_copy(f"bn{k}_t", ch[k - 1], Fk[k - 1]) if dec1_valu else None)
+            if f"bn{k}_t" in xh:
+                v = None
         vs[k] = v; dstats[k] = (mean, rstd); us[k - 1] = u
     if ups:
         uus[1] = ops.upsample_w(u, rows * ch[1], Fk[1], 2).view(B, T, ch[1], Fk[0])
@@ -644,7 +659,7 @@
                                  prec=prec)
     _flush_counters()
     if save:
-        ctx.update(ys=ys, es=es, stats=stats, gctx=gctx, us=us, vs=vs, dstats=dstats, mask=mask, uus=uus, dec_mode=dec_mode)
+        ctx.update(ys=ys, es=es, stats=stats, gctx=gctx, us=us, vs=vs, dstats=dstats, mask=mask, uus=uus, dec_mode=dec_mode, xh16=xh)
         if e_bf is not None and e_bf.dtype == torch.bfloat16:
             ctx["e_bf"] = e_bf.view(B, T, ch[L], Fk[L])
     return mask.view(B, ch[0], T, F0), ctx
@@ -675,6 +690,7 @@
     dy_bf16 = bool(config.get().bf16_dy) and ops.prec_code(prec) == ops.PREC_BF16 and dprec == ops.PREC_BF16 and all_mfma
     ups = ctx.get("dec_mode", "transposed") == "upsample"
     uus = ctx.get("uus", {})
+    xh = ctx.get("xh16", {})
 
     def dec_wgrad(k, dv_):
         if ups and ch[k - 1] % 4 != 0:
@@ -715,7 +731,7 @@
 
     def lvl_bf16(k):
         return de_bf16 and 2 <= k < L
-    du, du_sums = dec_dgrad(1, dv, bn_of(2, True) if L >= 2 else None)
+    du, du_sums = dec_dgrad(1, dv, bn_of(2, True) if L >= 2 and "bn2_t" not in xh else None)
     ds = {1: du}
     de_pre = {}
 
@@ -754,7 +770,7 @@
         else:
             dv = ops.bn_act_bwd(du, vs[k], mean, rstd, P[f"bn{k}_t.weight"], P[f"bn{k}_t.bias"], rows, ch[k - 1],
                                 Fk[k - 1], True, training, G[f"bn{k}_t.weight"], G[f"bn{k}_t.bias"],
-                                dbias=G.get(f"conv{k}_t.bias"), sums=du_sums, out_bf16=dy_bf16)
+                                dbias=G.get(f"conv{k}_t.bias"), sums=du_sums, out_bf16=dy_bf16, xh16=xh.get(f"bn{k}_t"))
 
         def leaf_dec(dv=dv, k=k):
             dec_wgrad(k, dv)
@@ -791,7 +807,7 @@
         else:
             dy = ops.bn_act_bwd(de, ys[k], mean, rstd, P[f"bn{k}.weight"], P[f"bn{k}.bias"], rows, ch[k], Fk[k], True,
                                 training, G[f"bn{k}.weight"], G[f"bn{k}.bias"], dbias=G[f"conv{k}.bias"], sums=de_sums,
-                                out_bf16=dy_bf16 and not (need_dx and k == 1))
+                                out_bf16=dy_bf16 and not (need_dx and k == 1), xh16=xh.get(f"bn{k}"))
 
         def leaf_enc(dy=dy, k=k):
             ops.conv_wgrad(dy, es[k - 1], G[f"conv{k}.weight"], B, T, ch[k], Fk[k], ch[k - 1], Fk[k - 1], KT=2, S=2, pad=1, prec=prec)
diff --git a/cruse_amd/ops.py b/cruse_amd/ops.py
--- a/cruse_amd/ops.py
+++ b/cruse_amd/ops.py
@@ -363,8 +363,17 @@
 BN_STAT_REPLICAS = 16
 
 
+def xh16_eligible(C, F) -> bool:
+    return (C * F) % 4 == 0 and C * F <= 768 and C <= 256
+
+
+def xh16_decode(xh16):
+    w = xh16.view(torch.int16)
+    return (w & -2).view(torch.float16).float(), (w & 1).bool()
+
+
 def bn_finalize_act_fwd(y, sums, count, eps, momentum, gamma, beta, skip, rows, C, F, relu=True, running_mean=None,
-                        running_var=None, out_bf16=None):
+                        running_var=None, out_bf16=None, xh16=None):
     if sums.numel() % (2 * C) != 0:
         raise RuntimeError(f"bn_finalize_act_fwd: {sums.numel()} sums for {C} channels")
     out = torch.empty_like(y)
@@ -372,9 +381,11 @@
     rstd = torch.empty(C, device=y.device, dtype=torch.float32)
     if out_bf16 is not None and (out_bf16.dtype not in (torch.bfloat16, torch.float16) or out_bf16.numel() < y.numel()):
         raise RuntimeError("bn_finalize_act_fwd: out_bf16 must be a bf16 (or f16) tensor of at least y.numel() elements")
-    check(lib.cruse_bn_finalize_act_fwd_c(_p(y), _p(sums), sums.numel() // (2 * C), count, eps, momentum, _p(gamma), _p(beta), _p(skip), _p(out),
-                                          _p(out_bf16), _copy_dt(out_bf16), _p(mean), _p(rstd), _p(running_mean), _p(running_var), rows, C, F,
-                                          1 if relu else 0, _stream()))
+    if xh16 is not None and (xh16.dtype != torch.int16 or xh16.numel() != y.numel() or not xh16.is_contiguous()):
+        raise RuntimeError("bn_finalize_act_fwd: xh16 must be a contiguous int16 tensor of y.numel() elements")
+    check(lib.cruse_bn_finalize_act_fwd_x16(_p(y), _p(sums), sums.numel() // (2 * C), count, eps, momentum, _p(gamma), _p(beta), _p(skip), _p(out),
+                                            _p(out_bf16), _copy_dt(out_bf16), _p(xh16), _p(mean), _p(rstd), _p(running_mean), _p(running_var),
+                                            rows, C, F, 1 if relu else 0, _stream()))
     return out, mean, rstd
 
 
@@ -402,7 +413,9 @@
 
 
 def bn_act_bwd(dout, y, mean, rstd, gamma, beta, rows, C, F, relu, training, dgamma, dbeta, dbias=None, sums=None,
-               out_bf16=False):
+               out_bf16=False, xh16=None):
+    if xh16 is not None:
+        return _bn_act_bwd_x16(dout, xh16, rstd, gamma, rows, C, F, relu, training, dgamma, dbeta, dbias, sums, out_bf16)
     nrep = BN_STAT_REPLICAS
     if sums is None:
         nrep = 1
@@ -415,6 +428,22 @@
                                      1 if relu else 0, 1 if training else 0, _xdt(dout, "bn_act_bwd dout"), _p(dy), 2 if out_bf16 else 0,
                                      _p(dgamma), _p(dbeta),
                                      _p(dbias), _stream()))
+    return dy
+
+
+def _bn_act_bwd_x16(dout, xh16, rstd, gamma, rows, C, F, relu, training, dgamma, dbeta, dbias, sums, out_bf16):
+    if xh16.dtype != torch.int16 or xh16.numel() != rows * C * F or not training:
+        raise RuntimeError("bn_act_bwd: xh16 must be the int16 copy of this BatchNorm's input, written in training mode")
+    nrep = BN_STAT_REPLICAS
+    if sums is None:
+        nrep = 1
+        sums, z = ARENA.take(2 * C, xh16.device)
+        _f32(dout, "bn_act_bwd (reduce pass) dout")
+        check(lib.cruse_bn_act_bwd_reduce_x16(_p(dout), _p(xh16), rows, C, F, 1 if relu else 0, _p(sums), z, _stream()))
+    dy = torch.empty(dout.shape, device=dout.device, dtype=torch.bfloat16 if out_bf16 else torch.float32)
+    check(lib.cruse_bn_act_bwd_apply_x16(_p(dout), _p(xh16), _p(rstd), _p(gamma), _p(sums), nrep, rows, C, F, 1 if relu else 0, 1,
+                                         _xdt(dout, "bn_act_bwd dout"), _p(dy), 2 if out_bf16 else 0, _p(dgamma), _p(dbeta), _p(dbias),
+                                         _stream()))
     return dy
 
 
diff --git a/include/cruse_hip.h b/include/cruse_hip.h
--- a/include/cruse_hip.h
+++ b/include/cruse_hip.h
@@ -135,6 +135,16 @@
                            const float* gamma, const float* beta, const double* sums, int sum_replicas,
                            long long rows, int C, int F, int relu, int training, int dout_dtype,
                            void* dy, int dy_dtype, float* dgamma, float* dbeta, float* dbias, void* stream);
+
+int cruse_bn_finalize_act_fwd_x16(const float* y, const double* sums, int sum_replicas, long long count, float eps, float momentum,
+                                  const float* gamma, const float* beta, const float* skip, float* out, void* out_copy, int copy_dtype,
+                                  void* xh16, float* mean, float* rstd, float* running_mean, float* running_var,
+                                  long long rows, int C, int F, int relu, void* stream);
+int cruse_bn_act_bwd_reduce_x16(const float* dout, const void* xh16, long long rows, int C, int F, int relu, double* sums, int zeroed,
+                                void* stream);
+int cruse_bn_act_bwd_apply_x16(const void* dout, const void* xh16, const float* rstd, const float* gamma, const double* sums,
+                               int sum_replicas, long long rows, int C, int F, int relu, int training, int dout_dtype,
+                               void* dy, int dy_dtype, float* dgamma, float* dbeta, float* dbias, void* stream);
 
 
 int cruse_ln_fwd(const float* x, const float* gamma, const float* beta, const float* res,
```
